# chellmuth/pathed

Measured on AMD Instinct MI355X. Metric: Msamples/s (pixels x spp / s), PathTracer radiance loop, higher is better.
Workload: dtype f32; 1 GPU; scenes/cornell.json 1024x1024, 1024 spp per step x 8 steps = 8192 spp, bounces 0..10, seed 1; total_samples=8589934592, parallelism=the samples of every step split over 1 GPU(s), no exchange

## Files before the change

pathed_amd/csrc/kernels.h:

```cpp
#pragma once

#ifndef PATHED_RESOLVE_SHARED
#define PATHED_RESOLVE_SHARED 2
#endif
#ifndef PATHED_EXPERIMENTS
#define PATHED_EXPERIMENTS 0
#endif
#include "mfma_candidates.h"
#include "small_items.h"
#include "camera_masks.h"
#include "shading.h"
#include "trace.h"
#include "volume.h"

namespace pathed {

static const int kBlock = 256;
static_assert(kBlock == kVolumeBlock, "volume.h indexes the LDS stack rows with the block size");
static const int kWavesPerBlock = kBlock / 64;
static const int kMaxLdsMaterials = 96;
#ifndef PATHED_UNIT_QUEUES
#define PATHED_UNIT_QUEUES 32
#endif
static const int kUnitQueues = PATHED_UNIT_QUEUES;
// ... 1115 lines not shown
                target = (unsigned int)floatAsInt(sd.w);
                valid = true;
            }
        }
        if (__ballot(valid) == 0ull) { continue; }

        unsigned int candidatesLow = 0, candidatesHigh = 0;
        if (valid) {
            smallCandidates<true>(smallTris.data, nTris, ray.o, ray.d, &candidatesLow, &candidatesHigh,
                                  candidateNear(ray.tnear), ray.anyHit ? candidateFar(ray.tfar) : 3e38f);
            if (COUNT) { trisTested += (unsigned int)nTris; }
        }

        smallResolve(geometry, ray, candidatesLow, candidatesHigh);

        if (valid) {
            finishRay(geometry, ray);
            if (ray.anyHit) {
                if (ray.occluded) { p.state.pend[target] = make_float4(0.f, 0.f, 0.f, 0.f); }
                if (COUNT) { shadowRays++; }
            } else {
                p.state.hit[target] = make_float4(ray.best, ray.bestU, ray.bestV, intAsFloat(ray.bestPrim));
                if (COUNT) { closestRays++; }
            }
        }
    }

    if (COUNT) {
        atomicAdd(&p.stats[kStatTris], (unsigned long long)trisTested);
        atomicAdd(&p.stats[kStatClosest], (unsigned long long)closestRays);
        atomicAdd(&p.stats[kStatShadow], (unsigned long long)shadowRays);
    }
}

template <int STACK, int FORMAT>
__global__ __launch_bounds__(kBlock) void k_trace_rays(
    DScene scene, const float4 *rays, int n, int anyHit, float4 *hitsOut, int *occludedOut,
    int *stackOverflow, int maxStack
) {
    extern __shared__ float4 ldsRaw[];
    LaneStack stack;
    stack.lds = reinterpret_cast<int *>(ldsRaw) + threadIdx.x;
    stack.overflowStride = (size_t)gridDim.x * kBlock;
    stack.overflow = stackOverflow + ((size_t)blockIdx.x * kBlock + threadIdx.x);

    TraceGeometry geometry;
    geometry.nodes = FORMAT != 0 ? scene.nodesQ : scene.nodes;
    geometry.tris = scene.leafTris;
    geometry.nNodes = scene.nNodes;
    geometry.nTris = scene.nTris;
    geometry.spheres = scene.spheres;
    geometry.nSpheres = scene.nLinearSpheres;

    const int i = blockIdx.x * kBlock + threadIdx.x;
    if (i >= n) { return; }
    const float4 ro = rays[2 * i + 0];
    const float4 rd = rays[2 * i + 1];
    RayHit hit;
    hit.t = 0.f; hit.u = 0.f; hit.v = 0.f; hit.prim = -1;
    TraceCounters counters;
    if (anyHit) {
        const bool occluded = traverse<false, STACK, kBlock, FORMAT>(
            geometry, stack, maxStack, v3(ro.x, ro.y, ro.z), v3(rd.x, rd.y, rd.z), ro.w, rd.w, true, &hit, &counters);
        occludedOut[i] = occluded ? 1 : 0;
    } else {
        const bool found = traverse<false, STACK, kBlock, FORMAT>(
            geometry, stack, maxStack, v3(ro.x, ro.y, ro.z), v3(rd.x, rd.y, rd.z), ro.w, rd.w, false, &hit, &counters);
        if (!found) { hit.t = 0.f; hit.u = 0.f; hit.v = 0.f; hit.prim = -1; }
        hitsOut[i] = make_float4(hit.t, hit.u, hit.v, intAsFloat(hit.prim));
    }
}

template <int STACK, bool COUNT>
__global__ __launch_bounds__(kBlock) void k_trace_instanced(RenderParams p, DInstanceSet instances)
{
    extern __shared__ float4 ldsRaw[];
    LaneStack stack;
    stack.lds = reinterpret_cast<int *>(ldsRaw) + threadIdx.x;
    stack.overflowStride = (size_t)gridDim.x * kBlock;
    stack.overflow = p.stackOverflow + ((size_t)blockIdx.x * kBlock + threadIdx.x);

    TraceGeometry geometry;
    geometry.nodes = p.scene.nodes;
    geometry.tris = p.scene.leafTris;
    geometry.nNodes = p.scene.nNodes;
    geometry.nTris = p.scene.nTris;
    geometry.spheres = nullptr;
    geometry.nSpheres = 0;

    const int lane = threadIdx.x & 63;
    const unsigned int waveId = blockIdx.x * kWavesPerBlock + (threadIdx.x >> 6);
    const unsigned int waveCount = gridDim.x * kWavesPerBlock;
    const unsigned int slotBatches = (unsigned int)p.nSlots / 64u;
    const unsigned int shadowCount = p.counters[kCtrShadowCount + (p.parity ^ 1) * kCursorStride];
    const unsigned int totalBatches = slotBatches + (shadowCount + 63u) / 64u;

    TraceCounters counters;
    counters.boxes = 0;
    counters.tris = 0;
    unsigned int closestRays = 0, shadowRays = 0;

    for (unsigned int batch = waveId; batch < totalBatches; batch += waveCount) {
        LaneRay ray;
        const float4 *worldO = nullptr, *worldD = nullptr;
        unsigned int target = 0;
        if (batch < slotBatches) {
            const unsigned int slot = batch * 64u + lane;
            const float4 rd = p.state.rayD[slot];
            if (!(floatAsInt(rd.w) & kStDone)) {
                const float4 ro = p.state.rayO[slot];
                laneRayInit(ray, v3(ro.x, ro.y, ro.z), v3(rd.x, rd.y, rd.z), PATHED_TNEAR, PATHED_TFAR, false);
                worldO = p.state.rayO + slot;
                worldD = p.state.rayD + slot;
                target = slot;
            }
        } else {
            const unsigned int entry = (batch - slotBatches) * 64u + lane;
            if (entry < shadowCount) {
                const float4 so = p.state.shO[entry];
                const float4 sd = p.state.shD[entry];
                laneRayInit(ray, v3(so.x, so.y, so.z), v3(sd.x, sd.y, sd.z), PATHED_TNEAR, so.w, true);
                worldO = p.state.shO + entry;
                worldD = p.state.shD + entry;
                target = (unsigned int)floatAsInt(sd.w);
            }
        }
        if (worldO == nullptr) { continue; }
        traverseInstanced<COUNT, STACK, kBlock>(geometry, instances, stack, p.maxStack, worldO, worldD, ray, &counters);
        if (ray.anyHit) {
            if (ray.occluded) { p.state.pend[target] = make_float4(0.f, 0.f, 0.f, 0.f); }
            if (COUNT) { shadowRays++; }
        } else {
            p.state.hit[target] = make_float4(ray.best, ray.bestU, ray.bestV, intAsFloat(ray.bestPrim));
            if (COUNT) { closestRays++; }
        }
    }

    if (COUNT) {
        atomicAdd(&p.stats[kStatBoxes], (unsigned long long)counters.boxes);
        atomicAdd(&p.stats[kStatTris], (unsigned long long)counters.tris);
        atomicAdd(&p.stats[kStatClosest], (unsigned long long)closestRays);
        atomicAdd(&p.stats[kStatShadow], (unsigned long long)shadowRays);
    }
}

template <int STACK>
__global__ __launch_bounds__(kBlock) void k_trace_rays_instanced(
    DScene scene, DInstanceSet instances, const float4 *rays, int n, int anyHit, float4 *hitsOut, int *occludedOut,
    int *stackOverflow, int maxStack
) {
    extern __shared__ float4 ldsRaw[];
    LaneStack stack;
    stack.lds = reinterpret_cast<int *>(ldsRaw) + threadIdx.x;
    stack.overflowStride = (size_t)gridDim.x * kBlock;
    stack.overflow = stackOverflow + ((size_t)blockIdx.x * kBlock + threadIdx.x);

    TraceGeometry geometry;
    geometry.nodes = scene.nodes;
    geometry.tris = scene.leafTris;
    geometry.nNodes = scene.nNodes;
    geometry.nTris = scene.nTris;
    geometry.spheres = nullptr;
    geometry.nSpheres = 0;

    const int i = blockIdx.x * kBlock + threadIdx.x;
    if (i >= n) { return; }
    const float4 ro = rays[2 * i + 0];
    const float4 rd = rays[2 * i + 1];
    TraceCounters counters;
    LaneRay ray;
    laneRayInit(ray, v3(ro.x, ro.y, ro.z), v3(rd.x, rd.y, rd.z), ro.w, rd.w, anyHit != 0);
    traverseInstanced<false, STACK, kBlock>(geometry, instances, stack, maxStack, rays + 2 * i, rays + 2 * i + 1, ray, &counters);
    if (anyHit) {
        occludedOut[i] = ray.occluded ? 1 : 0;
    } else if (ray.bestPrim >= 0) {
        hitsOut[i] = make_float4(ray.best, ray.bestU, ray.bestV, intAsFloat(ray.bestPrim));
    } else {
        hitsOut[i] = make_float4(0.f, 0.f, 0.f, intAsFloat(-1));
    }
}


__device__ inline V3 triangleNormal(V3 p0, V3 p1, V3 p2) { return normalized(xcross(p1 - p0, p2 - p0)); }

template <typename TRAITS = TraitsAll, bool INSTANCED = false>
__device__ inline Isect makeIsect(const DScene &scene, V3 o, V3 d, float4 h, const DInstanceSet *instances = nullptr)
{
    const float t = h.x, u = h.y, v = h.z;
#if defined(PATHED_ABLATE) && PATHED_ABLATE == 1
    const int prim = floatAsInt(h.w) & 1023;
#else
    const int prim = floatAsInt(h.w);
#endif

    V3 geometricNormal;
    V3 shadingNormal = v3(0.f, 0.f, 0.f);
    float uvU = 0.f, uvV = 0.f;
    int material;

    if (INSTANCED && prim >= instances->worldTris) {
        int low = 0, high = instances->nInstances - 1;
        while (low < high) {
            const int middle = (low + high + 1) >> 1;
            if (instances->bases[middle] <= prim) { low = middle; } else { high = middle - 1; }
        }
        const float4 *record = instances->records + (size_t)kInstanceQuads * low;
        const float4 m0 = record[0], m1 = record[1], m2 = record[2], i0 = record[3], i1 = record[4], i2 = record[5], ids = record[6];
        const float m[12] = { m0.x, m0.y, m0.z, m0.w, m1.x, m1.y, m1.z, m1.w, m2.x, m2.y, m2.z, m2.w };
        const float inverse[12] = { i0.x, i0.y, i0.z, i0.w, i1.x, i1.y, i1.z, i1.w, i2.x, i2.y, i2.z, i2.w };
        const float4 *q = scene.triShade + (size_t)kTriShadeQuads * (size_t)(floatAsInt(ids.w) + (prim - floatAsInt(ids.x)));
        const float4 q0 = q[0], q1 = q[1], q2 = q[2], q3 = q[3], q4 = q[4], q5 = q[5], q6 = q[6];
        const V3 p0 = flattenPoint(m, v3(q0.x, q0.y, q0.z)), p1 = flattenPoint(m, v3(q1.x, q1.y, q1.z)), p2 = flattenPoint(m, v3(q2.x, q2.y, q2.z));
        const V3 n0 = flattenNormal(inverse, v3(q3.x, q3.y, q3.z)), n1 = flattenNormal(inverse, v3(q4.x, q4.y, q4.z)), n2 = flattenNormal(inverse, v3(q5.x, q5.y, q5.z));
        const float w = 1.f - u - v;
        uvU = fmaf(w, q1.w, fmaf(u, q3.w, v * q5.w));
        uvV = fmaf(w, q2.w, fmaf(u, q4.w, v * q6.x));
        shadingNormal = v3(
            fmaf(w, n0.x, fmaf(u, n1.x, v * n2.x)),
            fmaf(w, n0.y, fmaf(u, n1.y, v * n2.y)),
            fmaf(w, n0.z, fmaf(u, n1.z, v * n2.z)));
        geometricNormal = triangleNormal(p0, p1, p2);
        material = floatAsInt(q0.w);
        if (length(shadingNormal) == 0.f) { shadingNormal = geometricNormal; }
        shadingNormal = normalized(shadingNormal);
    } else if (!TRAITS::spheres || prim < scene.nTris) {
        bool plain = false;
        for (int r = 0; r < scene.nPlainRanges; r++) { plain = plain || (prim >= scene.plainBegin[r] && prim < scene.plainEnd[r]); }
        if (plain) {
            const float4 *c = scene.triCompact + (size_t)kTriCompactQuads * prim;
            const float4 c0 = c[0], c1 = c[1];
            material = floatAsInt(c0.w);
            geometricNormal = v3(c0.x, c0.y, c0.z);
            shadingNormal = v3(c1.x, c1.y, c1.z);
        } else {
            const float4 *q = scene.triShade + (size_t)kTriShadeQuads * prim;
            const float4 q0 = q[0], q1 = q[1], q2 = q[2], q3 = q[3], q4 = q[4], q5 = q[5], q6 = q[6];
            const V3 p0 = v3(q0.x, q0.y, q0.z), p1 = v3(q1.x, q1.y, q1.z), p2 = v3(q2.x, q2.y, q2.z);
            const float w = 1.f - u - v;
            uvU = fmaf(w, q1.w, fmaf(u, q3.w, v * q5.w));
            uvV = fmaf(w, q2.w, fmaf(u, q4.w, v * q6.x));
            shadingNormal = v3(
                fmaf(w, q3.x, fmaf(u, q4.x, v * q5.x)),
                fmaf(w, q3.y, fmaf(u, q4.y, v * q5.y)),
                fmaf(w, q3.z, fmaf(u, q4.z, v * q5.z)));
            geometricNormal = triangleNormal(p0, p1, p2);
            material = floatAsInt(q0.w);
            if (length(shadingNormal) == 0.f) { shadingNormal = geometricNormal; }
            shadingNormal = normalized(shadingNormal);
        }
    } else {
        const DSphere sphere = scene.spheres[prim - scene.nTris];
        const V3 point = o + d * t;
        geometricNormal = normalized(point - v3(sphere.centerWorld[0], sphere.centerWorld[1], sphere.centerWorld[2]));
        material = sphere.material;
        shadingNormal = normalized(geometricNormal);
    }

    Isect isect;
    isect.point = o + d * t;
    isect.wo = -d;
    isect.normal = geometricNormal;
    isect.shadingNormal = shadingNormal;
    isect.u = uvU;
    isect.v = uvV;
    isect.material = material;
    isect.prim = prim;
    isect.frame = normalToWorldSpace(isect.shadingNormal, isect.wo);
    isect.woLocal = v3(__builtin_nanf(""), __builtin_nanf(""), __builtin_nanf(""));
    return isect;
}

template <typename TRAITS = TraitsAll>
__device__ inline float lightsPDF(const DScene &scene, V3 referencePoint, const Isect &lightIsect)
{
    float measurePDF;
    if (!TRAITS::spheres || lightIsect.prim < scene.nTris) {
        const float4 q7 = scene.triShade[(size_t)kTriShadeQuads * lightIsect.prim + 7];
        measurePDF = areaToSolidAngle(q7.w, referencePoint, lightIsect.point, v3(q7.x, q7.y, q7.z));
    } else {
        const DSphere sphere = scene.spheres[lightIsect.prim - scene.nTris];
        measurePDF = spherePdfSolidAngle(
            v3(sphere.centerSample[0], sphere.centerSample[1], sphere.centerSample[2]), sphere.radius, referencePoint);
    }
    return measurePDF / scene.nLights;
}

template <typename TRAITS = TraitsAll>
__device__ inline Rgb environmentL(const DScene &scene, V3 direction)
{
    if (!TRAITS::env) { return rgb(0.f); }
#if defined(PATHED_ABLATE) && PATHED_ABLATE == 3
    return rgb(0.f);
#endif
    if (scene.hasEnv) { return envEmit(scene.env, -direction); }
    return rgb(0.f);
}

struct ShadowRequest {
    bool push;
    V3 origin, direction;
    float tfar;
};

template <bool ENV_ONLY = false, typename TRAITS = TraitsAll, typename MaterialTable>
__device__ inline Rgb sampleLightsTerm(
    const DScene &scene, const MaterialTable &materials,
    const Isect &isect, const DMaterial &material, Rng &random, ShadowRequest *shadow
) {
    shadow->push = false;
#if defined(PATHED_ABLATE) && PATHED_ABLATE == 2
    return rgb(0.f);
#endif
    if (isDeltaT<TRAITS>(material)) { return rgb(0.f); }
    if (scene.nLights == 0) { return rgb(0.f); }

    const int lightCount = ENV_ONLY ? 1 : scene.nLights;
    DLight light;
    light.kind = 2;
    light.index = 0;
    int lightIndex = 0;
    if (ENV_ONLY) {
        random.dimension++;
    } else {
        lightIndex = (int)floorf(random.next() * lightCount);
        lightIndex = imin(lightIndex, lightCount - 1);
        light = scene.lights[lightIndex];
    }

    SurfaceSample surfaceSample;
    int lightMaterial = 0;
    constexpr bool kRecords = !ENV_ONLY && TRAITS::triangleLights && !TRAITS::spheres && !TRAITS::env;
    float pdfArea = 0.f;
    if (ENV_ONLY) {
        surfaceSample = envSample<TRAITS::pairedTrig>(scene.env, isect.point, random);
    } else if (!kRecords && TRAITS::triangleLights && light.kind == 0) {
        const float4 *q = scene.triShade + (size_t)kTriShadeQuads * light.index;
        const float4 q0 = q[0], q1 = q[1], q2 = q[2];
        surfaceSample = triangleSample(v3(q0.x, q0.y, q0.z), v3(q1.x, q1.y, q1.z), v3(q2.x, q2.y, q2.z), random);
        lightMaterial = floatAsInt(q0.w);
    } else if (kRecords) {
        const float4 *l = scene.lightRecords + (size_t)kLightRecordQuads * lightIndex;
        const float4 l0 = l[0], l1 = l[1], l2 = l[2];
        surfaceSample = triangleSamplePoint(v3(l0.x, l0.y, l0.z), v3(l1.x, l1.y, l1.z), v3(l2.x, l2.y, l2.z), v3(0.f, 0.f, 0.f), l1.w, random);
        __builtin_amdgcn_sched_barrier(0);
        const float4 l3 = l[3];
        surfaceSample.normal = v3(l3.x, l3.y, l3.z);
        lightMaterial = floatAsInt(l0.w);
        pdfArea = l3.w;
    } else if (TRAITS::spheres && (light.kind == 1 || !TRAITS::env)) {
        const DSphere sphere = scene.spheres[light.index];
        surfaceSample = sphereSample<TRAITS::pairedTrig>(
            v3(sphere.centerSample[0], sphere.centerSample[1], sphere.centerSample[2]), sphere.radius, isect.point, random);
        lightMaterial = sphere.material;
    } else if (TRAITS::env) {
        surfaceSample = envSample<TRAITS::pairedTrig>(scene.env, isect.point, random);
    } else {
        surfaceSample.point = isect.point;
        surfaceSample.normal = v3(0.f, 0.f, 0.f);
        surfaceSample.invPDF = 1.f;
        surfaceSample.solidAngle = 1;
    }
    const float lightChoicePDF = 1.f / lightCount;
    const float invPDF = surfaceSample.invPDF * (1.f / lightChoicePDF);
    if (!kRecords) { pdfArea = 1.f / invPDF; }

    const V3 lightDirection = surfaceSample.point - isect.point;
    const V3 wiWorld = normalized(lightDirection);

    if (dot(surfaceSample.normal, wiWorld) >= 0.f) { return rgb(0.f); }

    const float lightDistance = length(lightDirection);

    float pdf;
    if (surfaceSample.solidAngle) {
        pdf = pdfArea;
    } else {
        const V3 lightWoForPdf = -normalized(lightDirection);
        const float distance2 = lightDistance * lightDistance;
        const float projectedArea = smax(0.f, dot(surfaceSample.normal, lightWoForPdf));
        pdf = pdfArea * distance2 / projectedArea;
    }

    float brdfPDF;
    const Rgb f = materialF<TRAITS>(material, isect, wiWorld, &brdfPDF);
    const float lightWeight = (1 * pdf) / (1 * pdf + 1 * brdfPDF);

    if (isBlack(f) && pdf > 0.f && pdf < 3e38f && brdfPDF >= 0.f && brdfPDF < 3e38f) { return rgb(0.f); }

    const V3 lightWo = -normalized(lightDirection);
    Rgb emitted;
    if (ENV_ONLY || (TRAITS::env && light.kind == 2)) { emitted = envEmit(scene.env, lightWo); }
    else { emitted = matEmit(materials[lightMaterial]); }

    shadow->push = true;
    shadow->origin = isect.point;
    shadow->direction = wiWorld;
    shadow->tfar = lightDistance - 1e-3f;

    const Rgb contribution = emitted
        * lightWeight
        * f
        * fabsf(dot(isect.shadingNormal, wiWorld))
        / pdf;
    return contribution;
}

__device__ inline void startSample(const RenderParams &p, uint32_t pixel, uint32_t sample, int sampleInUnit, float4 *rayO, float4 *rayD)
{
    const int width = p.scene.camera.resX;
    const int row = (int)fastDivide((unsigned int)pixel, p.divWidth);
    const int col = (int)pixel - row * width;
    Rng random;
    makeKey(((uint64_t)p.seedHi << 32) | p.seedLo, pixel, sample, &random.k0, &random.k1);
    random.dimension = 0;
    const float jitterX = random.next() - 0.5f;
    const float jitterY = random.next() - 0.5f;
    V3 origin, direction;
    cameraRay(p.scene.camera, row + jitterY, col + jitterX, &origin, &direction);
    *rayO = make_float4(origin.x, origin.y, origin.z, intAsFloat(-1));
    *rayD = make_float4(direction.x, direction.y, direction.z, intAsFloat(sampleInUnit << kStSampleShift));
}

__device__ inline unsigned int grabUnits(const RenderParams &p, bool want, unsigned int *ldsScratch)
{
    const int lane = threadIdx.x & 63;
    const int wave = threadIdx.x >> 6;
    const unsigned int queues = (unsigned int)p.nQueues;
    const unsigned int home = blockIdx.x % queues;
    unsigned int mine = 0xFFFFFFFFu;
    for (unsigned int attempt = 0; attempt < queues; attempt++) {
        const unsigned long long mask = __ballot(want);
        const unsigned int before = (unsigned int)__popcll(mask & ((1ull << lane) - 1ull));
        if (lane == 0) { ldsScratch[wave] = (unsigned int)__popcll(mask); }
        __syncthreads();
        unsigned int offset = 0, total = 0;
        #pragma unroll
        for (int w = 0; w < kWavesPerBlock; w++) {
            const unsigned int count = ldsScratch[w];
            if (w < wave) { offset += count; }
            total += count;
        }
        if (total == 0u) { __syncthreads(); break; }
        const unsigned int queue = (unsigned int)__builtin_amdgcn_readfirstlane((int)(home + attempt < queues ? home + attempt : home + attempt - queues));
        const unsigned int limit = p.queueUnits[queue];
        if (threadIdx.x == 0) {
            unsigned int *cursor = &p.counters[kCtrUnitCursor + queue * kCursorStride];
            const unsigned int seen = __atomic_load_n(cursor, __ATOMIC_RELAXED);
            ldsScratch[kWavesPerBlock] = seen < limit ? atomicAdd(cursor, total) : 0xFFFFFFFFu;
        }
        __syncthreads();
        const unsigned int base = ldsScratch[kWavesPerBlock];
        __syncthreads();
        if (base >= limit) { continue; }
        if (want) {
            const unsigned int k = base + offset + before;
            if (k < limit) { mine = queue * p.unitsPerQueue + k; want = false; }
        }
        if (base + total <= limit) { break; }
    }
    return mine;
}

static const int kOrderStripes = 0, kOrderStripesTiled = 1, kOrderTiles = 2, kOrderList = 3;

__device__ inline unsigned int tileWalkPixel(const RenderParams &p, unsigned int index)
{
    const unsigned int width = (unsigned int)p.scene.camera.resX, height = (unsigned int)p.scene.camera.resY;
    const unsigned int band = fastDivide(index, p.divBand);
    const unsigned int inBand = index - band * 8u * width;
    const unsigned int rowsLeft = height - 8u * band;
    const unsigned int rows = rowsLeft < 8u ? rowsLeft : 8u;
    const unsigned int block = rows == 8u ? inBand >> 8 : inBand / (32u * rows);
    const unsigned int inBlock = inBand - block * 32u * rows;
    const unsigned int columnsLeft = width - 32u * block;
    const unsigned int columns = columnsLeft < 32u ? columnsLeft : 32u;
    const unsigned int y = columns == 32u ? inBlock >> 5 : inBlock / columns;
    const unsigned int x = inBlock - y * columns;
    return (8u * band + y) * width + 32u * block + x;
}

__device__ inline const uint32_t *pixelList(const RenderParams &p) { return reinterpret_cast<const uint32_t *>(p.cameraQueue); }

template <bool LIST = false>
__device__ inline void unitPlace(const RenderParams &p, unsigned int unit, uint32_t *pixel, uint32_t *chunkIndex)
{
    const unsigned int queue = fastDivide(unit, p.divStride);
    const unsigned int k = unit - queue * p.unitsPerQueue;
    const unsigned int j = fastDivide(k, p.divGroupUnits);
    const unsigned int w = k - j * p.groupUnits;
    const unsigned int owned = queue * p.pools + p.pool + j * (unsigned int)p.nQueues * p.pools;
    if (p.unitOrder != kOrderTiles) {
        *chunkIndex = owned;
        if constexpr (LIST) {
            if (p.unitOrder == kOrderStripes) { *pixel = w; }
            else if (p.unitOrder == kOrderList) { *pixel = pixelList(p)[w]; }
            else { *pixel = tileWalkPixel(p, w); }
        } else {
            *pixel = p.unitOrder == kOrderStripes ? w : tileWalkPixel(p, w);
        }
        return;
    }
    unsigned int chunk, within;
    if (owned + 1u < p.nGroups || p.lastGroupPixels == kUnitGroup) {
        chunk = w >> 8;
        within = w & (kUnitGroup - 1u);
    } else {
        chunk = w / p.lastGroupPixels;
        within = w - chunk * p.lastGroupPixels;
    }
    *pixel = tileWalkPixel(p, owned * kUnitGroup + within);
    *chunkIndex = chunk;
}

template <bool LIST = false>
__device__ inline void unitSamples(const RenderParams &p, unsigned int unit, uint32_t *pixel, uint32_t *first, uint32_t *end)
{
    uint32_t chunkIndex;
    unitPlace<LIST>(p, unit, pixel, &chunkIndex);
    *first = p.sppBegin + chunkIndex * (unsigned int)p.chunk;
    const uint32_t last = *first + (unsigned int)p.chunk;
    *end = last < p.sppEnd ? last : p.sppEnd;
}

template <bool LIST = false>
__device__ inline size_t partialIndex(const RenderParams &p, unsigned int unit)
{
    uint32_t pixel, chunkIndex;
    unitPlace<LIST>(p, unit, &pixel, &chunkIndex);
    return (size_t)chunkIndex * (size_t)p.nPixels + pixel;
}

__global__ __launch_bounds__(kBlock) void k_init(RenderParams p)
{
    __shared__ unsigned int scratch[kWavesPerBlock + 1];
    const int slot = blockIdx.x * kBlock + threadIdx.x;
    const unsigned int unit = grabUnits(p, true, scratch);

    float4 rayO = make_float4(0.f, 0.f, 0.f, intAsFloat(-1));
    float4 rayD = make_float4(0.f, 0.f, 0.f, intAsFloat(kStDone));
    const bool started = unit != 0xFFFFFFFFu;
    if (started) {
        uint32_t pixel, first, end;
        unitSamples<true>(p, unit, &pixel, &first, &end);
        startSample(p, pixel, first, 0, &rayO, &rayD);
    }
    p.state.rayO[slot] = rayO;
    p.state.rayD[slot] = rayD;
    p.state.res[slot] = make_float4(0.f, 0.f, 0.f, intAsFloat((int)unit));
    p.state.mod[slot] = make_float4(1.f, 1.f, 1.f, 1.f);
    p.state.thr[slot] = make_float4(0.f, 0.f, 0.f, 0.f);
    p.state.pend[slot] = make_float4(0.f, 0.f, 0.f, 0.f);
    p.state.acc[slot] = make_float4(0.f, 0.f, 0.f, 0.f);

    const unsigned long long mask = __ballot(started);
    if ((threadIdx.x & 63) == 0 && mask != 0ull) {
        atomicAdd(&p.counters[kCtrRemaining], (unsigned int)__popcll(mask));
    }
}

__global__ __launch_bounds__(kBlock) void k_resolve(RenderParams p)
{
    const int pixel = blockIdx.x * kBlock + threadIdx.x;
    if (pixel >= p.nPixels) { return; }
    float *out = p.accum + 3 * (size_t)pixel;
    float r = out[0], g = out[1], b = out[2];
    int chunk = 0;
    for (; chunk + 8 <= p.chunksPerPixel; chunk += 8) {
        float4 partial[8];
        #pragma unroll
        for (int k = 0; k < 8; k++) { partial[k] = p.state.chunkBuf[(size_t)(chunk + k) * p.nPixels + pixel]; }
        #pragma unroll
        for (int k = 0; k < 8; k++) {
            r += partial[k].x;
            g += partial[k].y;
            b += partial[k].z;
        }
    }
    for (; chunk < p.chunksPerPixel; chunk++) {
        const float4 partial = p.state.chunkBuf[(size_t)chunk * p.nPixels + pixel];
        r += partial.x;
        g += partial.y;
        b += partial.z;
    }
    out[0] = r;
    out[1] = g;
    out[2] = b;
}

struct MomentsParams {
    const float4 *chunkBuf;
    int nPixels;
    int chunksPerPixel;
    float *sum;
    float *squares;
};

__global__ __launch_bounds__(kBlock) void k_resolve_moments(MomentsParams p)
{
    const int pixel = blockIdx.x * kBlock + threadIdx.x;
    if (pixel >= p.nPixels) { return; }
    float *out = p.sum + 3 * (size_t)pixel;
    float *outSquares = p.squares + 3 * (size_t)pixel;
    float r = out[0], g = out[1], b = out[2];
    float rr = outSquares[0], gg = outSquares[1], bb = outSquares[2];
    int chunk = 0;
    for (; chunk + 8 <= p.chunksPerPixel; chunk += 8) {
        float4 partial[8];
        #pragma unroll
        for (int k = 0; k < 8; k++) { partial[k] = p.chunkBuf[(size_t)(chunk + k) * p.nPixels + pixel]; }
        #pragma unroll
// ... 725 lines not shown

    ShadowRequest shadow;
    shadow.push = false;
    shadow.origin = v3(0.f, 0.f, 0.f);
    shadow.direction = v3(0.f, 0.f, 0.f);
    shadow.tfar = 0.f;

    bool finished = false;
    Rgb color = rgb(0.f);
    unsigned int unit = 0xFFFFFFFFu;
    int sampleInUnit = 0;
    float4 outRayO = make_float4(0.f, 0.f, 0.f, 0.f), outRayD = rd;
    float4 outMod = make_float4(1.f, 1.f, 1.f, 1.f);
    float4 outThr = make_float4(0.f, 0.f, 0.f, 0.f);
    float4 outPend = make_float4(0.f, 0.f, 0.f, 0.f);
    Rgb result = rgb(0.f);
    V3 o = v3(0.f, 0.f, 0.f), d = v3(0.f, 0.f, 1.f);
    float4 hitNow = h;
    int rayBounce = 0, firstEmitMaterial = -1;
    uint32_t pixel = 0, sample = 0;
    bool haveVertex = false;
    bool hitWritten = false;
    float4 localHit = make_float4(PATHED_TFAR, 0.f, 0.f, intAsFloat(-1));

    unsigned int countedClosest = 0u, countedShadow = 0u;

    SHADE_REGION(0, true);
    SHADE_REGION(1, active);
    if (active) {
        const float4 ro = roIn;
        const float4 resIn = resIn0;
        outRayO = ro;
        o = v3(ro.x, ro.y, ro.z);
        d = v3(rd.x, rd.y, rd.z);
        rayBounce = st & kStBounceMask;
        sampleInUnit = (st >> kStSampleShift) & kStSampleMask;
        const bool miss = floatAsInt(h.w) < 0;
        unit = (unsigned int)floatAsInt(resIn.w);
        firstEmitMaterial = floatAsInt(ro.w);
        uint32_t firstSample, endSample;
        unitSamples<true>(p, unit, &pixel, &firstSample, &endSample);
        sample = firstSample + (uint32_t)sampleInUnit;
        result = rgb(resIn.x, resIn.y, resIn.z);
        Rgb modulation = rgb(1.f);
        Rgb missLight = rgb(0.f);
        if (miss && (rayBounce == 0 || (st & kStEligible))) { missLight = environmentL<TRAITS>(scene, d); }

        if (rayBounce == 0) {
            if (miss) {
                color = rgb(0.f) + missLight;
                finished = true;
            } else {
                firstEmitMaterial = -1;
                result = rgb(0.f);
                haveVertex = true;
            }
        } else {
            const float4 modIn = p.state.mod[slot];
            const float4 thrIn = p.state.thr[slot];
            modulation = rgb(modIn.x, modIn.y, modIn.z);
            const float bsdfPdf = modIn.w;
            const Rgb throughput = rgb(thrIn.x, thrIn.y, thrIn.z);
            const float cosTheta = thrIn.w;
            if (st & kStEligible) {
                Rgb bsdfTerm = rgb(0.f);
                if (miss) {
                    const Rgb environmentLight = missLight;
                    if (!isBlack(environmentLight)) {
                        const float lightPDF = envEmitPDF(scene.env, d) / 1;
                        const float brdfWeight = (st & kStDelta)
                            ? 1.f
                            : (1 * bsdfPdf) / (1 * bsdfPdf + 1 * lightPDF);
                        bsdfTerm = environmentLight * brdfWeight * throughput * cosTheta / bsdfPdf;
                    }
                }
                const Rgb Ld = rgb(pendIn.x, pendIn.y, pendIn.z) + bsdfTerm;
                if (rayBounce == 1) { result = Ld; }
                else { result = result + Ld * modulation; }
            }
            if (!(st & kStContinue) || miss) {
                finished = true;
            } else {
                const float invPDF = 1.f / bsdfPdf;
                modulation = modulation * (throughput * cosTheta * invPDF);
                if (isBlack(modulation)) { finished = true; }
                else { haveVertex = true; }
            }
            if (finished) {
                const Rgb first = rgb(0.f);
                color = first + result;
            }
        }
        outMod = make_float4(modulation.r, modulation.g, modulation.b, 1.f);
    }

    bool retiredAny = false;
#define PATHED_END_OF_SAMPLE(ended, value, startedNext, nextPixel, nextSample)                                                 \
    {                                                                                                                        \
        bool needUnit_ = false;                                                                                              \
        startedNext = false;                                                                                                 \
        SHADE_REGION(7, ended);                                                                                              \
        if (ended) {                                                                                                         \
            const bool singleSample_ = PATHED_SHADE_TRIM && p.chunk == 1;                                                    \
            float4 partial_ = make_float4(0.f, 0.f, 0.f, 0.f);                                                               \
            if (!singleSample_) { partial_ = p.state.acc[slot]; }                                                            \
            const bool finite_ = isfinite((value).r) && isfinite((value).g) && isfinite((value).b);                          \
            if (finite_) {                                                                                                   \
                partial_.x += (value).r;                                                                                     \
                partial_.y += (value).g;                                                                                     \
                partial_.z += (value).b;                                                                                     \
            } else {                                                                                                         \
                atomicAdd(&p.stats[kStatDropped], 1ull);                                                                     \
            }                                                                                                                \
            uint32_t unitPixel_, firstSample_, endSample_;                                                                   \
            unitSamples<true>(p, unit, &unitPixel_, &firstSample_, &endSample_);                                             \
            sampleInUnit++;                                                                                                  \
            result = rgb(0.f);                                                                                               \
            outMod = make_float4(1.f, 1.f, 1.f, 1.f);                                                                        \
            outThr = make_float4(0.f, 0.f, 0.f, 0.f);                                                                        \
            outPend = make_float4(0.f, 0.f, 0.f, 0.f);                                                                       \
            if (firstSample_ + (uint32_t)sampleInUnit < endSample_) {                                                        \
                startedNext = true;                                                                                          \
                nextPixel = unitPixel_;                                                                                      \
                nextSample = firstSample_ + (uint32_t)sampleInUnit;                                                          \
                p.state.acc[slot] = partial_;                                                                                \
            } else {                                                                                                         \
                p.state.chunkBuf[partialIndex<true>(p, unit)] = partial_;                                                    \
                if (!singleSample_) { p.state.acc[slot] = make_float4(0.f, 0.f, 0.f, 0.f); }                                 \
                needUnit_ = true;                                                                                            \
            }                                                                                                                \
        }                                                                                                                    \
        const unsigned int newUnit_ = grabUnits(p, needUnit_, scratch);                                                      \
        if (needUnit_) {                                                                                                     \
            unit = newUnit_;                                                                                                 \
            if (newUnit_ != 0xFFFFFFFFu) {                                                                                   \
                uint32_t endSample_;                                                                                         \
                unitSamples<true>(p, newUnit_, &nextPixel, &nextSample, &endSample_);                                        \
                sampleInUnit = 0;                                                                                            \
                startedNext = true;                                                                                          \
            } else {                                                                                                         \
                outRayD.w = intAsFloat(kStDone);                                                                             \
                retiredAny = true;                                                                                           \
            }                                                                                                                \
        }                                                                                                                    \
        SHADE_REGION(8, startedNext);                                                                                        \
        if (startedNext) { startSample(p, nextPixel, nextSample, sampleInUnit, &outRayO, &outRayD); }                        \
    }

    {
        bool startedNext;
        uint32_t nextPixel = 0, nextSample = 0;
        PATHED_END_OF_SAMPLE(active && finished, color, startedNext, nextPixel, nextSample)
        if (p.localCount > 0) {
            const V3 cameraO = v3(outRayO.x, outRayO.y, outRayO.z), cameraD = v3(outRayD.x, outRayD.y, outRayD.z);
            const bool localCamera = startedNext && !localMeetsRest(p, cameraO, cameraD, PATHED_TFAR);
            const float4 found = localClosestHit(p, localCamera, cameraO, cameraD);
            if (localCamera) {
                countedClosest++;
                if (floatAsInt(found.w) >= 0) {
                    o = cameraO; d = cameraD; hitNow = found;
                    rayBounce = 0; firstEmitMaterial = -1;
                    pixel = nextPixel; sample = nextSample;
                    result = rgb(0.f);
                    haveVertex = true;
                } else {
                    localHit = found;
                    hitWritten = true;
                    outRayD.w = intAsFloat(floatAsInt(outRayD.w) | kStLocal);
                }
            }
        }
    }

    SHADE_REGION(5, haveVertex);
    if (haveVertex) {
        Isect isect = makeIsect<TRAITS>(scene, o, d, hitNow);
        const int vertex = rayBounce + 1;
        const DMaterial &material = materials[isect.material];
        prepareLobes<TRAITS>(material, isect);
        Rng random;
        makeKey(((uint64_t)p.seedHi << 32) | p.seedLo, pixel, sample, &random.k0, &random.k1);
        random.dimension = vertexBase(vertex);
        const BSDFSample bsdfSample = materialSample<TRAITS>(material, isect, random);

        const bool counts = checkCounts(p.startBounce, p.lastBounce, vertex);
        const bool wantDirect = counts;
        const bool wantContinue = !checkDone(p.lastBounce, vertex + 1);

        Rgb lightTerm = rgb(0.f);
        SHADE_REGION(6, wantDirect);
        if (wantDirect) {
            random.dimension = vertexBase(vertex) + 3;
            lightTerm = sampleLightsTerm<true, TRAITS>(scene, materials, isect, material, random, &shadow);
        }
        const bool deadEnd = isBlack(bsdfSample.throughput) && bsdfSample.pdf > 0.f && bsdfSample.pdf < 3e38f
            && !shadow.push && isBlack(lightTerm);
        if ((!wantDirect && !wantContinue) || deadEnd) {
            outRayO = make_float4(isect.point.x, isect.point.y, isect.point.z, intAsFloat(firstEmitMaterial));
            outRayD = make_float4(d.x, d.y, d.z, intAsFloat((vertex | (sampleInUnit << kStSampleShift)) | kStLocal));
            outMod.w = 1.f;
            outThr = make_float4(0.f, 0.f, 0.f, 0.f);
            outPend = make_float4(0.f, 0.f, 0.f, 0.f);
            localHit = make_float4(PATHED_TFAR, 0.f, 0.f, intAsFloat(-1));
            hitWritten = true;
            shadow.push = false;
        } else {
            int nextState = vertex | (sampleInUnit << kStSampleShift);
            if (wantDirect) { nextState |= kStEligible; }
            if (isDeltaT<TRAITS>(material)) { nextState |= kStDelta; }
            if (wantContinue) { nextState |= kStContinue; }
            outRayO = make_float4(isect.point.x, isect.point.y, isect.point.z, intAsFloat(firstEmitMaterial));
            outRayD = make_float4(bsdfSample.wiWorld.x, bsdfSample.wiWorld.y, bsdfSample.wiWorld.z, intAsFloat(nextState));
            if (rayBounce == 0) { outMod = make_float4(1.f, 1.f, 1.f, 1.f); }
            outMod.w = bsdfSample.pdf;
            outThr = make_float4(
                bsdfSample.throughput.r, bsdfSample.throughput.g, bsdfSample.throughput.b,
                fabsf(dot(isect.shadingNormal, bsdfSample.wiWorld)));
            outPend = make_float4(lightTerm.r, lightTerm.g, lightTerm.b, 0.f);
            hitWritten = false;
        }
    }
#undef PATHED_END_OF_SAMPLE

    if (p.localCount > 0) {
        const bool retiredNow = (floatAsInt(outRayD.w) & kStDone) != 0;
        const bool hasRay = active && !retiredNow;
        const V3 nextO = v3(outRayO.x, outRayO.y, outRayO.z), nextD = v3(outRayD.x, outRayD.y, outRayD.z);
        const bool localClosest = hasRay && !hitWritten && !localMeetsRest(p, nextO, nextD, PATHED_TFAR);
        const bool localShadow = shadow.push && !localMeetsRest(p, shadow.origin, shadow.direction, shadow.tfar);
        {
            const float4 found = localClosestHit(p, localClosest, nextO, nextD);
            if (localClosest) {
                localHit = found;
                hitWritten = true;
                outRayD.w = intAsFloat(floatAsInt(outRayD.w) | kStLocal);
                countedClosest++;
            }
            const bool occluded = localOccluded(p, localShadow, shadow.origin, shadow.direction, shadow.tfar);
            if (localShadow) {
                if (occluded) { outPend = make_float4(0.f, 0.f, 0.f, 0.f); }
                shadow.push = false;
                countedShadow++;
            }
        }
        if (hasRay && (!(floatAsInt(outRayD.w) & kStLocal) || shadow.push)) { outRayD.w = intAsFloat(floatAsInt(outRayD.w) | kStAwait); }
        if (p.localCounting) {
            for (int offset = 32; offset >= 1; offset >>= 1) {
                countedClosest += (unsigned int)__shfl_xor((int)countedClosest, offset, 64);
                countedShadow += (unsigned int)__shfl_xor((int)countedShadow, offset, 64);
            }
            if (lane == 0 && (countedClosest | countedShadow) != 0u) {
                atomicAdd(&p.stats[kStatLocalClosest], (unsigned long long)countedClosest);
                atomicAdd(&p.stats[kStatLocalShadow], (unsigned long long)countedShadow);
            }
        }
    }

    if (active) {
        p.state.rayO[slot] = outRayO;
        p.state.rayD[slot] = outRayD;
        p.state.res[slot] = make_float4(result.r, result.g, result.b, intAsFloat((int)unit));
        if (hitWritten) { p.state.hit[slot] = localHit; }
        p.state.mod[slot] = outMod;
        p.state.thr[slot] = outThr;
        p.state.pend[slot] = outPend;
    }

    {
        const unsigned long long mask = __ballot(shadow.push);
        const unsigned int before = (unsigned int)__popcll(mask & ((1ull << lane) - 1ull));
        if (lane == 0) { scratch[wave] = (unsigned int)__popcll(mask); }
        __syncthreads();
        unsigned int offset = 0, total = 0;
        #pragma unroll
        for (int w = 0; w < kWavesPerBlock; w++) {
            const unsigned int count = scratch[w];
            if (w < wave) { offset += count; }
            total += count;
        }
        __syncthreads();
        if (threadIdx.x == 0) {
            scratch[kWavesPerBlock] = total ? atomicAdd(&p.counters[kCtrShadowCount + p.parity * kCursorStride], total) : 0u;
        }
        __syncthreads();
        if (shadow.push) {
            const unsigned int index = scratch[kWavesPerBlock] + offset + before;
            p.state.shO[index] = make_float4(shadow.origin.x, shadow.origin.y, shadow.origin.z, shadow.tfar);
            p.state.shD[index] = make_float4(shadow.direction.x, shadow.direction.y, shadow.direction.z, intAsFloat(slot));
        }
    }

    const unsigned long long retiredMask = __ballot(retiredAny);
    if (lane == 0 && retiredMask != 0ull) {
        atomicSub(&p.counters[kCtrRemaining], (unsigned int)__popcll(retiredMask));
    }
}

#ifndef PATHED_FUSED_WAVES
#define PATHED_FUSED_WAVES 4
#endif
template <bool LDS_MATERIALS, bool COUNT, typename TRAITS, bool MFMA = false, bool QUADS = false>
__global__ __launch_bounds__(kBlock) __attribute__((amdgpu_waves_per_eu(PATHED_FUSED_WAVES, PATHED_FUSED_WAVES))) void k_path_small(RenderParams p, SmallTris smallTris)
{
    extern __shared__ float4 ldsDynamic[];
    __shared__ float mfmaRows[MFMA ? kMfmaTableFloats : 1];
    __shared__ float4 stashRows[QUADS ? 6 * kBlock : 1];
    constexpr int kResolveCapacity = PATHED_RESOLVE_SHARED == 2 ? 128 : 64;
    __shared__ unsigned long long resolveBest[QUADS ? kBlock : 1];
    __shared__ float2 resolveUv[QUADS ? kWavesPerBlock * kResolveCapacity : 1];
    __shared__ unsigned short resolveItems[QUADS ? kWavesPerBlock * kResolveCapacity : 1];
    __shared__ unsigned int resolveOccluded[QUADS ? kBlock : 1], resolveCount[QUADS ? kWavesPerBlock : 1];
    if (MFMA) {
        for (int i = threadIdx.x; i < kMfmaTableFloats; i += kBlock) { mfmaRows[i] = p.mfmaTable[i]; }
        if (!LDS_MATERIALS) { __syncthreads(); }
    }
    const MaterialAccess<LDS_MATERIALS> materials = stageMaterials<LDS_MATERIALS>(p, ldsDynamic);
    const TraceGeometry geometry = sceneGeometry(p.scene, false);

    const DScene &scene = p.scene;
    const int lane = threadIdx.x & 63;
    const unsigned int waveId = blockIdx.x * kWavesPerBlock + (unsigned int)__builtin_amdgcn_readfirstlane((int)(threadIdx.x >> 6));
    const int nTris = p.scene.nTris;
    constexpr bool kPassList = QUADS && kSmallPassList<COUNT, MFMA, TRAITS>;
    TraceGeometry passGeometry = geometry;
    if (kPassList) { passGeometry.tris = geometry.tris + 3 * nTris; }
    const uint64_t seed = ((uint64_t)p.seedHi << 32) | p.seedLo;
    UnitTaker units(p, waveId);

    bool alive = true;
    bool needEntry = true;
    unsigned int unit = 0xFFFFFFFFu;
    uint32_t pixel = 0, sample = 0, endSample = 0;
    PathRegisters path = idlePath();
    float4 partial = make_float4(0.f, 0.f, 0.f, 0.f);
    bool pendingShadow = false;
    V3 shadowDirection = v3(0.f, 0.f, 1.f);
    float shadowTfar = 0.f;

    unsigned int closestRays = 0, shadowRays = 0, trisTested = 0;

    float4 *const cameraQueue = p.cameraQueue + (size_t)waveId * kCameraQueueWords;
    unsigned int queueHead = 0u, queueCount = 0u;
    bool unitsLeft = true;
    const bool singleSample = p.chunk == 1;

    bool startNext = false;

    while (true) {
        SHADE_REGION(0, alive && !needEntry);
        SHADE_REGION(1, startNext);
        if (startNext) {
            startCameraSample(p, seed, pixel, sample, path);
            startNext = false;
        }

        if (QUADS) {
            float4 *stash = stashRows + threadIdx.x;
            stash[0 * kBlock] = make_float4(path.result.r, path.result.g, path.result.b, path.bsdfPdf);
            stash[1 * kBlock] = make_float4(path.modulation.r, path.modulation.g, path.modulation.b, path.cosTheta);
            stash[2 * kBlock] = make_float4(path.throughput.r, path.throughput.g, path.throughput.b, intAsFloat(path.st));
            stash[3 * kBlock] = partial;
            stash[4 * kBlock] = make_float4(intAsFloat((int)pixel), intAsFloat((int)sample), intAsFloat((int)endSample), intAsFloat((int)unit));
            stash[5 * kBlock] = make_float4(intAsFloat((int)path.random.k0), intAsFloat((int)path.random.k1), intAsFloat(path.firstEmitMaterial), intAsFloat((int)path.random.dimension));
            asm volatile("" ::: "memory");
        }

        if (queueCount < 64u && unitsLeft) {
            const unsigned int newUnit = units.take(p, lane, true);
            const bool got = newUnit != 0xFFFFFFFFu;
            const unsigned long long gotMask = __ballot(got);
            SHADE_REGION(11, got);
            if (gotMask != ~0ull) { unitsLeft = false; }
            Rng cameraRandom;
            cameraRandom.k0 = 0u; cameraRandom.k1 = 0u; cameraRandom.dimension = 0u;
            V3 cameraO = v3(0.f, 0.f, 0.f), cameraD = v3(0.f, 0.f, 1.f);
            constexpr bool kMasks = !COUNT && !MFMA;
            uint32_t unitPixel = 0u;
            if (got) {
                uint32_t unitFirst, unitEnd;
                unitSamples(p, newUnit, &unitPixel, &unitFirst, &unitEnd);
                cameraSampleRay(p, seed, unitPixel, unitFirst, cameraRandom, &cameraO, &cameraD);
            }
            LaneRay cameraHit;
            laneRayInit(cameraHit, cameraO, cameraD, PATHED_TNEAR, PATHED_TFAR, false);
            unsigned int candidatesLow = 0, candidatesHigh = 0;
            if (kMasks) {
                if (got) {
                    const unsigned long long pixelCandidates = cameraMasks(p)[unitPixel];
                    candidatesLow = (unsigned int)(pixelCandidates >> 32);
                    candidatesHigh = (unsigned int)pixelCandidates;
                }
            } else if (got) {
                if (QUADS || MFMA) {
                    unsigned int unusedLow = 0, unusedHigh = 0;
                    smallCandidatesItems<false, true, true>(smallTris.data, p.smallQuads, nTris, p.smallKappaT, cameraO, cameraD, cameraD,
                                                             &candidatesLow, &candidatesHigh, &unusedLow, &unusedHigh, candidateNear(PATHED_TNEAR), 0.f);
                } else {
                    smallCandidates(smallTris.data, nTris, cameraO, cameraD, &candidatesLow, &candidatesHigh, candidateNear(PATHED_TNEAR));
                }
            }
            if (COUNT && got) {
                trisTested += (unsigned int)nTris;
                closestRays++;
            }
            smallResolve(geometry, cameraHit, candidatesLow, candidatesHigh);
            if (got) {
                finishRay(geometry, cameraHit);
                const unsigned int slot = (queueHead + queueCount + laneRank(gotMask)) & (kCameraQueueEntries - 1u);
                const unsigned int target = singleSample ? (unsigned int)partialIndex(p, newUnit) : newUnit;
                cameraQueue[0 * kCameraQueueEntries + slot] = make_float4(cameraD.x, cameraD.y, cameraD.z, cameraHit.best);
                cameraQueue[1 * kCameraQueueEntries + slot] = make_float4(cameraHit.bestU, cameraHit.bestV, intAsFloat(cameraHit.bestPrim), intAsFloat((int)target));
                cameraQueue[2 * kCameraQueueEntries + slot] = make_float4(intAsFloat((int)cameraRandom.k0), intAsFloat((int)cameraRandom.k1), 0.f, 0.f);
            }
            queueCount += (unsigned int)__popcll(gotMask);
            __threadfence_block();
        }

        const bool tracing = alive && !needEntry;
        LaneRay ray;
        laneRayInit(ray, path.o, path.d, PATHED_TNEAR, PATHED_TFAR, false);
        {
            const bool traceShadow = tracing && pendingShadow;
            LaneRay shadowRay;
            laneRayInit(shadowRay, path.o, shadowDirection, PATHED_TNEAR, shadowTfar, true);
            unsigned int candidatesLow = 0, candidatesHigh = 0, shadowLow = 0, shadowHigh = 0;
            SHADE_REGION(2, traceShadow);
            if (MFMA) {
                mfmaCandidatesPair(mfmaRows, nTris, p.mfmaFrame, __ballot(traceShadow) != 0ull, path.o, path.d, shadowDirection,
                                   candidateNear(PATHED_TNEAR), candidateFar(shadowTfar), &candidatesLow, &candidatesHigh, &shadowLow, &shadowHigh);
                if (!tracing) { candidatesLow = 0u; candidatesHigh = 0u; }
                if (!traceShadow) { shadowLow = 0u; shadowHigh = 0u; }
            } else if (QUADS) {
                if (tracing) {
                    constexpr bool kPrune = kSmallPrunes<COUNT, TRAITS>;
                    const int smallQuads = kPassList ? (p.smallQuads & 0xFF) : kPrune ? (p.smallQuads & 0xFFFF) : p.smallQuads;
                    const int passTris = kPassList ? ((p.smallQuads >> 8) & 0xFF) : nTris;
                    smallCandidatesItems<true, true, true, kPrune>(smallTris.data, smallQuads, passTris, p.smallKappaT, path.o, path.d, shadowDirection,
                                                                   &candidatesLow, &candidatesHigh, &shadowLow, &shadowHigh,
                                                                   candidateNear(PATHED_TNEAR), candidateFar(shadowTfar),
                                                                   (p.smallQuads >> 16) & 0xFF, (p.smallQuads >> 24) & 0xFF);
                    if (!traceShadow) { shadowLow = 0u; shadowHigh = 0u; }
                }
            } else if (__ballot(traceShadow) != 0ull) {
                if (tracing) {
                    smallCandidatesPair(smallTris.data, nTris, path.o, path.d, shadowDirection, &candidatesLow, &candidatesHigh, &shadowLow, &shadowHigh,
                                        candidateNear(PATHED_TNEAR), candidateFar(shadowTfar));
                    if (!traceShadow) { shadowLow = 0u; shadowHigh = 0u; }
                }
            } else if (tracing) {
                smallCandidates(smallTris.data, nTris, path.o, path.d, &candidatesLow, &candidatesHigh, candidateNear(PATHED_TNEAR));
            }
            if (COUNT && tracing) {
                trisTested += (unsigned int)nTris * (traceShadow ? 2u : 1u);
                closestRays++;
                if (traceShadow) { shadowRays++; }
            }
            bool spheresDone = false;
            RESOLVE_PROBE(9, candidatesLow, candidatesHigh);
            RESOLVE_PROBE(10, shadowLow, shadowHigh);
            if (MFMA) {
                mfmaResolve(geometry, ray, candidatesLow, candidatesHigh);
                mfmaResolve(geometry, shadowRay, shadowLow, shadowHigh);
            } else if (QUADS && PATHED_RESOLVE_SHARED) {
                ResolveScratch scratch;
                const int waveBase = (int)(threadIdx.x & ~63u), wave = (int)(threadIdx.x >> 6);
                scratch.best = resolveBest + waveBase; scratch.uv = resolveUv + wave * kResolveCapacity; scratch.items = resolveItems + wave * kResolveCapacity;
                scratch.occluded = resolveOccluded + waveBase; scratch.count = resolveCount + wave;
                unsigned int sphereCandidates = 0u, shadowSphereCandidates = 0u;
                if (TRAITS::spheres && geometry.nSpheres > 0 && tracing) {
                    smallSphereCandidates(p, geometry.nSpheres, path.o, path.d, shadowDirection, &sphereCandidates, &shadowSphereCandidates);
                    if (!traceShadow) { shadowSphereCandidates = 0u; }
                }
                spheresDone = smallResolveShared<kResolveCapacity, PATHED_RESOLVE_SHARED != 2, TRAITS::spheres>(
                    passGeometry, ray, shadowRay, candidatesLow, candidatesHigh, shadowLow, shadowHigh, sphereCandidates, shadowSphereCandidates, scratch);
            } else {
                smallResolve(passGeometry, ray, candidatesLow, candidatesHigh);
                smallResolve(passGeometry, shadowRay, shadowLow, shadowHigh);
            }
            if (tracing && !spheresDone) { finishRay(geometry, ray); }
            if (traceShadow) {
                if (!spheresDone) { finishRay(geometry, shadowRay); }
                if (shadowRay.occluded) { path.pend = rgb(0.f); }
            }
            pendingShadow = false;
        }
        if (QUADS) {
            asm volatile("" ::: "memory");
            const float4 *stash = stashRows + threadIdx.x;
            const float4 s0 = stash[0 * kBlock], s1 = stash[1 * kBlock], s2 = stash[2 * kBlock], s4 = stash[4 * kBlock], s5 = stash[5 * kBlock];
            path.result = rgb(0.f); path.result.r = s0.x; path.result.g = s0.y; path.result.b = s0.z; path.bsdfPdf = s0.w;
            path.modulation.r = s1.x; path.modulation.g = s1.y; path.modulation.b = s1.z; path.cosTheta = s1.w;
            path.throughput.r = s2.x; path.throughput.g = s2.y; path.throughput.b = s2.z; path.st = floatAsInt(s2.w);
            partial = stash[3 * kBlock];
            pixel = (uint32_t)floatAsInt(s4.x); sample = (uint32_t)floatAsInt(s4.y); endSample = (uint32_t)floatAsInt(s4.z); unit = (unsigned int)floatAsInt(s4.w);
            path.random.k0 = (uint32_t)floatAsInt(s5.x); path.random.k1 = (uint32_t)floatAsInt(s5.y); path.firstEmitMaterial = floatAsInt(s5.z); path.random.dimension = (uint32_t)floatAsInt(s5.w);
        }
        float4 h = make_float4(ray.best, ray.bestU, ray.bestV, intAsFloat(ray.bestPrim));

        bool done = false;
        bool departs = false;
        Rgb color = rgb(0.f);
        if (tracing) {
            const bool miss = floatAsInt(h.w) < 0;
            Isect arrived;
            SHADE_REGION(3, !miss);
            if (!miss) { arrived = makeIsect<TRAITS>(scene, path.o, path.d, h); }
            done = pathArrive<TRAITS, true>(p, scene, materials, path, arrived, miss, &color);
            departs = !done;
        }

        while (true) {
            SHADE_REGION(8, done);
            {
                const bool unitDone = putSampleAway(p, singleSample, done, color, partial, unit, sample, endSample);
                needEntry = needEntry || unitDone;
                startNext = startNext || (done && !unitDone);
            }
            done = false;
            const unsigned long long wanting = __ballot(needEntry);
            if (wanting == 0ull) { break; }
            if (queueCount == 0u) {
                if (!unitsLeft && needEntry) { alive = false; needEntry = false; }
                break;
            }
            __threadfence_block();
            const unsigned int rank = laneRank(wanting);
            if (needEntry && rank < queueCount) {
                const unsigned int slot = (queueHead + rank) & (kCameraQueueEntries - 1u);
                const float4 e0 = cameraQueue[0 * kCameraQueueEntries + slot];
                const float4 e1 = cameraQueue[1 * kCameraQueueEntries + slot];
                const float4 e2 = cameraQueue[2 * kCameraQueueEntries + slot];
                resetPath(path);
                path.o = cameraOrigin(scene.camera);
                path.d = v3(e0.x, e0.y, e0.z);
                path.random.k0 = (uint32_t)floatAsInt(e2.x); path.random.k1 = (uint32_t)floatAsInt(e2.y); path.random.dimension = 2u;
                h = make_float4(e0.w, e1.x, e1.y, e1.z);
                unit = (unsigned int)floatAsInt(e1.w);
                if (singleSample) { sample = 0u; endSample = 1u; }
                else { unitSamples(p, unit, &pixel, &sample, &endSample); }
                needEntry = false;
                if (floatAsInt(h.w) < 0) {
                    color = cameraMissColor<TRAITS>(scene, path.d);
                    done = true;
                } else {
                    departs = true;
                }
            }
            const unsigned int wanted = (unsigned int)__popcll(wanting);
            const unsigned int taken = wanted < queueCount ? wanted : queueCount;
            queueHead = (queueHead + taken) & (kCameraQueueEntries - 1u);
            queueCount -= taken;
        }
        if (__ballot(alive) == 0ull) { break; }

        SHADE_REGION(6, departs);
        bool ended = false;
        if (departs) {
            Isect isect = makeIsect<TRAITS>(scene, path.o, path.d, h);
            ShadowRequest shadow;
            ended = pathDepart<TRAITS, true>(p, scene, materials, path, isect, &shadow, &color);
            if (shadow.push) {
                pendingShadow = true;
                shadowDirection = shadow.direction;
                shadowTfar = shadow.tfar;
            }
        }
        if (__ballot(ended) != 0ull) {
            SHADE_REGION(8, ended);
            const bool unitDone = putSampleAway(p, singleSample, ended, color, partial, unit, sample, endSample);
            needEntry = needEntry || unitDone;
            startNext = startNext || (ended && !unitDone);
        }
    }

    if (COUNT) {
        atomicAdd(&p.stats[kStatTris], (unsigned long long)trisTested);
        atomicAdd(&p.stats[kStatClosest], (unsigned long long)closestRays);
        atomicAdd(&p.stats[kStatShadow], (unsigned long long)shadowRays);
    }
}

#include "path_wave.h"
#include "path_hybrid.h"
static_assert(sizeof(RenderParams) + sizeof(SmallTris) <= 4096, "the fused kernels' arguments must fit the 4 KB kernarg segment");

__global__ __launch_bounds__(kBlock) void k_debug_small_candidates(DScene scene, SmallTris smallTris, SmallTris smallItems, int nQuads, float kappaT,
                                                                   const float4 *itemTris, const float *mfmaTable, MfmaFrame frame,
                                                                   const float *rays, int n, unsigned long long *out)
{
#if PATHED_EXPERIMENTS
    __shared__ float mfmaRows[kMfmaTableFloats];
    for (int i = threadIdx.x; i < kMfmaTableFloats; i += kBlock) { mfmaRows[i] = mfmaTable[i]; }
    __syncthreads();
#endif
    const int index = blockIdx.x * kBlock + threadIdx.x;
    const float *r = rays + (size_t)10 * index;
    const V3 o = v3(r[0], r[1], r[2]), dA = v3(r[3], r[4], r[5]), dB = v3(r[6], r[7], r[8]);
    const float tfarB = r[9];
    const int nTris = scene.nTris;

    unsigned int aLow, aHigh, bLow, bHigh;
    smallCandidatesPair(smallTris.data, nTris, o, dA, dB, &aLow, &aHigh, &bLow, &bHigh, candidateNear(PATHED_TNEAR), candidateFar(tfarB));
    unsigned int iaLow, iaHigh, ibLow, ibHigh;
    smallCandidatesItems<true>(smallItems.data, nQuads, nTris, kappaT, o, dA, dB, &iaLow, &iaHigh, &ibLow, &ibHigh, candidateNear(PATHED_TNEAR), candidateFar(tfarB));
    unsigned int evenA = 0u, oddA = 0u, evenB = 0u, oddB = 0u;
#if PATHED_EXPERIMENTS
    mfmaCandidatesPair(mfmaRows, nTris, frame, true, o, dA, dB, candidateNear(PATHED_TNEAR), candidateFar(tfarB), &evenA, &oddA, &evenB, &oddB);
#endif

    unsigned long long valuA = 0, valuB = 0, mfmaA = 0, mfmaB = 0, acceptA = 0, acceptB = 0, itemsA = 0, itemsB = 0;
    for (int k = 0; k < nTris; k++) {
        const float4 t0 = scene.leafTris[3 * k + 0], t1 = scene.leafTris[3 * k + 1], t2 = scene.leafTris[3 * k + 2];
        const unsigned long long bit = 1ull << (floatAsInt(t0.w) & 63);
        if (((k < 32 ? aLow : aHigh) >> (31 - (k & 31))) & 1u) { valuA |= bit; }
        if (((k < 32 ? bLow : bHigh) >> (31 - (k & 31))) & 1u) { valuB |= bit; }
        if ((((k & 1) ? oddA : evenA) >> (k >> 1)) & 1u) { mfmaA |= bit; }
        if ((((k & 1) ? oddB : evenB) >> (k >> 1)) & 1u) { mfmaB |= bit; }
        float t, u, v;
        if (intersectTriangle(o, dA, v3(t0.x, t0.y, t0.z), v3(t1.x, t1.y, t1.z), v3(t2.x, t2.y, t2.z), &t, &u, &v) && t > PATHED_TNEAR && t <= PATHED_TFAR) { acceptA |= bit; }
        if (intersectTriangle(o, dB, v3(t0.x, t0.y, t0.z), v3(t1.x, t1.y, t1.z), v3(t2.x, t2.y, t2.z), &t, &u, &v) && t > PATHED_TNEAR && t <= tfarB) { acceptB |= bit; }
        const unsigned long long itemBit = 1ull << (floatAsInt(itemTris[3 * k].w) & 63);
        if (((k < 32 ? iaLow : iaHigh) >> (31 - (k & 31))) & 1u) { itemsA |= itemBit; }
        if (((k < 32 ? ibLow : ibHigh) >> (31 - (k & 31))) & 1u) { itemsB |= itemBit; }
    }
    if (index < n) {
        unsigned long long *row = out + (size_t)8 * index;
        row[0] = valuA; row[1] = valuB; row[2] = mfmaA; row[3] = mfmaB; row[4] = acceptA; row[5] = acceptB; row[6] = itemsA; row[7] = itemsB;
    }
}

__global__ __launch_bounds__(kBlock) void k_debug_shadow_candidates(DScene scene, SmallTris smallItems, int nQuads, float kappaT, int shadowQuadPairs, int shadowLonePairs,
                                                                    const float4 *itemTris, const float *rays, int n, unsigned long long *out)
{
    const int index = blockIdx.x * kBlock + threadIdx.x;
    const float *r = rays + (size_t)10 * index;
    const V3 o = v3(r[0], r[1], r[2]), dA = v3(r[3], r[4], r[5]), dB = v3(r[6], r[7], r[8]);
    const float tfarB = r[9];
    const int nTris = scene.nTris;
    unsigned int aLow, aHigh, bLow, bHigh;
    smallCandidatesItems<true, true, true, true>(smallItems.data, nQuads, nTris, kappaT, o, dA, dB, &aLow, &aHigh, &bLow, &bHigh,
                                                 candidateNear(PATHED_TNEAR), candidateFar(tfarB), shadowQuadPairs, shadowLonePairs);
    unsigned long long candidates = 0, accepted = 0;
    for (int k = 0; k < nTris; k++) {
        const float4 t0 = itemTris[3 * k + 0], t1 = itemTris[3 * k + 1], t2 = itemTris[3 * k + 2];
        const unsigned long long bit = 1ull << (floatAsInt(t0.w) & 63);
        if (((k < 32 ? bLow : bHigh) >> (31 - (k & 31))) & 1u) { candidates |= bit; }
        float t, u, v;
        if (intersectTriangle(o, dB, v3(t0.x, t0.y, t0.z), v3(t1.x, t1.y, t1.z), v3(t2.x, t2.y, t2.z), &t, &u, &v) && t > PATHED_TNEAR && t <= tfarB) { accepted |= bit; }
    }
    if (index < n) { out[(size_t)2 * index] = candidates; out[(size_t)2 * index + 1] = accepted; }
}

__global__ __launch_bounds__(kBlock) void k_debug_pass_candidates(SmallTris passItems, int nQuads, int nPass, float kappaT, int shadowQuadPairs, int shadowLonePairs,
                                                                  const float4 *passTris, const float *rays, int n, unsigned long long *out)
{
    const int index = blockIdx.x * kBlock + threadIdx.x;
    const float *r = rays + (size_t)10 * index;
    const V3 o = v3(r[0], r[1], r[2]), dA = v3(r[3], r[4], r[5]), dB = v3(r[6], r[7], r[8]);
    const float tfarB = r[9];
    unsigned int aLow, aHigh, bLow, bHigh;
    smallCandidatesItems<true, true, true, true>(passItems.data, nQuads, nPass, kappaT, o, dA, dB, &aLow, &aHigh, &bLow, &bHigh,
                                                 candidateNear(PATHED_TNEAR), candidateFar(tfarB), shadowQuadPairs, shadowLonePairs);
    unsigned long long candidatesA = 0, candidatesB = 0;
    for (int k = 0; k < nPass; k++) {
        const unsigned long long bit = 1ull << (floatAsInt(passTris[3 * k].w) & 63);
        if (((k < 32 ? aLow : aHigh) >> (31 - (k & 31))) & 1u) { candidatesA |= bit; }
        if (((k < 32 ? bLow : bHigh) >> (31 - (k & 31))) & 1u) { candidatesB |= bit; }
    }
    if (index < n) { out[(size_t)2 * index] = candidatesA; out[(size_t)2 * index + 1] = candidatesB; }
}

template <bool QUADS = false, typename MaterialTable>
__device__ __forceinline__ bool volumeQuerySmall(const VolumeContext<MaterialTable> &c, const f2 *pairRecords, int smallQuads, float smallKappaT,
                                                 int mode, V3 o, V3 d, float tfar, RayHit *hit, VolumeEvents *eventsOut)
{
    LaneRay ray;
    const bool anyHit = mode == kQueryVolumeOccluded;
    laneRayInit(ray, o, d, PATHED_TNEAR, tfar, anyHit);
    VolumeEvents events;
    eventsClear(events);
    unsigned int low = 0u, high = 0u;
    if (QUADS) {
        unsigned int unusedLow = 0u, unusedHigh = 0u;
        smallCandidatesItems<true>(pairRecords, smallQuads, c.geometry.nTris, smallKappaT, o, d, d, &unusedLow, &unusedHigh, &low, &high,
                                   candidateNear(PATHED_TNEAR), anyHit ? candidateFar(tfar) : 3e38f);
    } else {
        smallCandidates<true>(pairRecords, c.geometry.nTris, o, d, &low, &high, candidateNear(PATHED_TNEAR), anyHit ? candidateFar(tfar) : 3e38f);
    }
    bool decided = false;
    while (__ballot((low | high) != 0u) != 0ull) {
        if ((low | high) != 0u) {
            int k;
            if (low != 0u) { k = __clz((int)low); low &= ~(0x80000000u >> k); }
            else { k = __clz((int)high); high &= ~(0x80000000u >> k); k += 32; }
            const float4 t0 = c.geometry.tris[3 * k + 0];
            const float4 t1 = c.geometry.tris[3 * k + 1];
            const float4 t2 = c.geometry.tris[3 * k + 2];
            float t, u, v;
            if (intersectTriangle(ray.o, ray.d, v3(t0.x, t0.y, t0.z), v3(t1.x, t1.y, t1.z), v3(t2.x, t2.y, t2.z), &t, &u, &v)) {
                if (volumeAccept(c, mode, ray, events, t, u, v, floatAsInt(t0.w))) { decided = true; low = 0u; high = 0u; }
            }
        }
    }
    if (!decided) {
        for (int i = 0; i < c.geometry.nSpheres; i++) {
            if (volumeSphere(c, mode, ray, events, i)) { break; }
        }
    }
    if (mode == kQueryVolumeClosest) { eventsClip(events, ray.best); }
    if (eventsOut) { *eventsOut = events; }
    if (anyHit) { return ray.occluded; }
    hit->t = ray.best;
    hit->u = ray.bestU;
    hit->v = ray.bestV;
    hit->prim = ray.bestPrim;
    return ray.bestPrim >= 0;
}


template <bool QUADS = false, typename MaterialTable>
__device__ __forceinline__ void volumeQueryPairSmall(const VolumeContext<MaterialTable> &c, const f2 *pairRecords, int smallQuads, float smallKappaT, V3 o,
                                                     bool wantA, int modeA, V3 dA, RayHit *hitA, bool *foundA, VolumeEvents *eventsA,
                                                     bool wantB, V3 dB, float tfarB, bool *occludedB, VolumeEvents *eventsB)
{
    unsigned int lowA = 0u, highA = 0u, lowB = 0u, highB = 0u;
    if (QUADS) {
        smallCandidatesItems<true>(pairRecords, smallQuads, c.geometry.nTris, smallKappaT, o, dA, dB, &lowA, &highA, &lowB, &highB,
                                   candidateNear(PATHED_TNEAR), candidateFar(tfarB));
    } else {
        smallCandidatesPair(pairRecords, c.geometry.nTris, o, dA, dB, &lowA, &highA, &lowB, &highB, candidateNear(PATHED_TNEAR), candidateFar(tfarB));
    }
    if (!wantA) { lowA = 0u; highA = 0u; }
    if (!wantB) { lowB = 0u; highB = 0u; }
    auto resolve = [&](int mode, LaneRay &ray, VolumeEvents &events, unsigned int low, unsigned int high, bool want) {
        bool decided = false;
        while (__ballot((low | high) != 0u) != 0ull) {
            if ((low | high) != 0u) {
                int k;
                if (low != 0u) { k = __clz((int)low); low &= ~(0x80000000u >> k); }
                else { k = __clz((int)high); high &= ~(0x80000000u >> k); k += 32; }
                const float4 t0 = c.geometry.tris[3 * k + 0];
                const float4 t1 = c.geometry.tris[3 * k + 1];
                const float4 t2 = c.geometry.tris[3 * k + 2];
                float t, u, v;
                if (intersectTriangle(ray.o, ray.d, v3(t0.x, t0.y, t0.z), v3(t1.x, t1.y, t1.z), v3(t2.x, t2.y, t2.z), &t, &u, &v)) {
                    if (volumeAccept(c, mode, ray, events, t, u, v, floatAsInt(t0.w))) { decided = true; low = 0u; high = 0u; }
                }
            }
        }
        if (want && !decided) {
            for (int i = 0; i < c.geometry.nSpheres; i++) {
                if (volumeSphere(c, mode, ray, events, i)) { break; }
            }
        }
    };
    {
        LaneRay ray;
        laneRayInit(ray, o, dA, PATHED_TNEAR, PATHED_TFAR, false);
        VolumeEvents events;
        eventsClear(events);
        resolve(modeA, ray, events, lowA, highA, wantA);
        if (modeA == kQueryVolumeClosest) { eventsClip(events, ray.best); }
        *eventsA = events;
        hitA->t = ray.best; hitA->u = ray.bestU; hitA->v = ray.bestV; hitA->prim = ray.bestPrim;
        *foundA = ray.bestPrim >= 0;
    }
    {
        LaneRay ray;
        laneRayInit(ray, o, dB, PATHED_TNEAR, tfarB, true);
        VolumeEvents events;
        eventsClear(events);
        resolve(kQueryVolumeOccluded, ray, events, lowB, highB, wantB);
        *eventsB = events;
        *occludedB = ray.occluded;
    }
}

#ifndef PATHED_VOLUME_WAVES
#define PATHED_VOLUME_WAVES 4
#endif
template <bool LDS_MATERIALS, int STACK, bool SMALL, typename TRAITS, bool QUADS, bool GRID, bool MULTI = false, bool LIST = false>
__device__ __forceinline__ void pathVolume(const RenderParams &p, const SmallTris &smallTris)
{
    extern __shared__ float4 ldsRaw[];
    const MaterialAccess<LDS_MATERIALS> materials = stageMaterials<LDS_MATERIALS>(p, ldsRaw + ((STACK + 1) * kBlock) / 4);

    const DScene &scene = p.scene;
    VolumeContext<MaterialAccess<LDS_MATERIALS>> context;
    context.geometry = sceneGeometry(scene, true);
    context.stack.lds = reinterpret_cast<int *>(ldsRaw) + threadIdx.x;
    context.stack.overflowStride = (size_t)gridDim.x * kBlock;
    context.stack.overflow = p.stackOverflow + ((size_t)blockIdx.x * kBlock + threadIdx.x);
    context.maxStack = p.maxStack;
    context.scene = &scene;
    context.materials = materials;
    context.primMedium = scene.primMedium;
    context.media = scene.media;

    const int lane = threadIdx.x & 63;
    const unsigned int waveId = blockIdx.x * kWavesPerBlock + (threadIdx.x >> 6);
    const uint64_t seed = ((uint64_t)p.seedHi << 32) | p.seedLo;

    UnitTaker units(p, waveId);

    auto query = [&](int mode, V3 origin, V3 direction, float tfar, RayHit *hit, VolumeEvents *events) -> bool {
        if constexpr (SMALL) { return volumeQuerySmall<QUADS>(context, (const f2 *)smallTris.data, p.smallQuads, p.smallKappaT, mode, origin, direction, tfar, hit, events); }
        else { return volumeQuery<STACK>(context, mode, origin, direction, tfar, hit, events); }
    };

    auto transmit = [&](int index, V3 pointA, V3 pointB) -> Rgb {
        if constexpr (GRID) {
            const DMedium &record = context.media[index];
            if (record.kind == kMediumGrid) {
                const float channel = gridTransmittance(scene.grids[record.grid], scene.gridData, pointA, pointB);
                return rgb(channel, channel, channel);
            }
        }
        return mediumTransmittance(context.media[index], pointA, pointB);
    };
    auto transmission = [&](V3 origin, V3 direction, const VolumeEvents &events, int medium) -> Rgb {
        if constexpr (GRID) { return rayTransmissionOver(transmit, origin, direction, events, medium); }
        else { return rayTransmission(context.media, origin, direction, events, medium); }
    };

    RayHit segmentHit;
    segmentHit.t = 0.f; segmentHit.u = 0.f; segmentHit.v = 0.f; segmentHit.prim = -1;
    bool segmentFound = false, segmentKnown = false;

    auto vertexLighting = [&](const Isect &isect, int medium, const DMaterial &material, const BSDFSample &bsdfSample, Rng &random,
                              bool direct, bool needSegment) -> Rgb {
        SHADE_REGION(5, direct);
        const bool lit = direct && material.type != PATHED_MAT_PASSTHROUGH && isBlack(matEmit(material));
        bool wantShadow = false;
        DLight light;
        light.kind = 0; light.index = 0;
        SurfaceSample surfaceSample;
        surfaceSample.point = isect.point; surfaceSample.normal = v3(0.f, 0.f, 0.f); surfaceSample.invPDF = 1.f; surfaceSample.solidAngle = 1;
        int lightMaterial = 0;
        float invPDF = 1.f, lightDistance = 0.f;
        V3 lightDirection = v3(0.f, 0.f, 0.f), wiWorld = bsdfSample.wiWorld;
        if (lit && !volumeIsDelta(material) && scene.nLights != 0) {
            const int lightCount = scene.nLights;
            int lightIndex = (int)floorf(random.next() * lightCount);
            lightIndex = imin(lightIndex, lightCount - 1);
            light = scene.lights[lightIndex];
            if (TRAITS::triangleLights && light.kind == 0) {
                const LightRecord record = loadLightRecord(scene.lightRecords, lightIndex);
                surfaceSample = triangleSamplePoint(record.p0, record.p1, record.p2, record.normal, record.area, random);
                lightMaterial = record.material;
            } else if (TRAITS::spheres && light.kind == 1) {
                const DSphere sphere = scene.spheres[light.index];
                surfaceSample = sphereSample<TRAITS::pairedTrig>(v3(sphere.centerSample[0], sphere.centerSample[1], sphere.centerSample[2]), sphere.radius, isect.point, random);
                lightMaterial = sphere.material;
            } else if (TRAITS::env) {
                surfaceSample = envSample<TRAITS::pairedTrig>(scene.env, isect.point, random);
            } else {
                surfaceSample.point = isect.point; surfaceSample.normal = v3(0.f, 0.f, 0.f); surfaceSample.invPDF = 1.f; surfaceSample.solidAngle = 1;
            }
            const float lightChoicePDF = 1.f / lightCount;
            invPDF = surfaceSample.invPDF * (1.f / lightChoicePDF);
            lightDirection = surfaceSample.point - isect.point;
            wiWorld = normalized(lightDirection);
            if (!(dot(surfaceSample.normal, wiWorld) >= 0.f)) {
                lightDistance = length(lightDirection);
                wantShadow = true;
            }
        }

        const bool wantClosest = lit || needSegment;
        const int closestMode = lit ? kQueryVolumeClosest : kQueryRegular;
        RayHit bounceHit;
        bounceHit.t = 0.f; bounceHit.u = 0.f; bounceHit.v = 0.f; bounceHit.prim = -1;
        bool found = false, occluded = false;
        VolumeEvents skipped, events;
        eventsClear(skipped);
        eventsClear(events);
        auto finishLight = [&]() -> Rgb {
            if (!wantShadow || occluded) { return rgb(0.f); }
            const Rgb transmittance = transmission(isect.point, wiWorld, events, medium);
            float pdf;
            if (surfaceSample.solidAngle) {
                pdf = 1.f / invPDF;
// ... 603 lines not shown
```

pathed_amd/csrc/path_common.h:

```cpp

template <bool LDS_MATERIALS>
__device__ __forceinline__ MaterialAccess<LDS_MATERIALS> stageMaterials(const RenderParams &p, void *lds)
{
    MaterialAccess<LDS_MATERIALS> materials;
    if (LDS_MATERIALS) {
        const int words = p.scene.nMaterials * (int)(sizeof(DMaterial) / 4);
        const int *source = reinterpret_cast<const int *>(p.scene.materials);
        int *target = reinterpret_cast<int *>(lds);
        for (int i = threadIdx.x; i < words; i += kBlock) { target[i] = source[i]; }
        __syncthreads();
        materials.table = reinterpret_cast<const DMaterial *>(lds);
    } else {
        materials.table = p.scene.materials;
    }
    return materials;
}

__device__ __forceinline__ TraceGeometry sceneGeometry(const DScene &scene, bool tree)
{
    TraceGeometry geometry;
    geometry.nodes = tree ? scene.nodes : nullptr;
    geometry.tris = scene.leafTris;
    geometry.nNodes = tree ? scene.nNodes : 0;
    geometry.nTris = scene.nTris;
    geometry.spheres = scene.spheres;
    geometry.nSpheres = scene.nLinearSpheres;
    return geometry;
}

struct UnitTaker {
    unsigned int queue, queuesTried;
    unsigned int reservedNext, reservedEnd;

    __device__ __forceinline__ UnitTaker(const RenderParams &p, unsigned int waveId)
        : queue(waveId % (unsigned int)p.nQueues), queuesTried(0), reservedNext(0), reservedEnd(0) {}

    __device__ __forceinline__ unsigned int take(const RenderParams &p, int lane, bool want)
    {
        unsigned int mine = 0xFFFFFFFFu;
        unsigned long long wanting = __ballot(want);
        while (wanting != 0ull) {
            if (reservedNext == reservedEnd) {
                if (queuesTried >= (unsigned int)p.nQueues) { break; }
                unsigned int ticket = 0;
                if (lane == 0) { ticket = atomicAdd(&p.counters[kCtrUnitCursor + queue * kCursorStride], (unsigned int)p.unitGrab); }
                ticket = (unsigned int)__builtin_amdgcn_readfirstlane((int)ticket);
                const unsigned int limit = p.queueUnits[queue];
                if (ticket >= limit) {
                    queue = (queue + 1u) % (unsigned int)p.nQueues;
                    queuesTried++;
                    continue;
                }
                reservedNext = ticket;
                reservedEnd = ticket + (unsigned int)p.unitGrab < limit ? ticket + (unsigned int)p.unitGrab : limit;
            }
            const unsigned int available = reservedEnd - reservedNext;
            const unsigned int rank = laneRank(wanting);
            const bool served = ((wanting >> lane) & 1ull) != 0ull && rank < available;
            if (served) { mine = queue * p.unitsPerQueue + reservedNext + rank; }
            const unsigned int count = (unsigned int)__popcll(wanting);
            reservedNext += count < available ? count : available;
            wanting &= ~__ballot(served);
        }
        return mine;
    }
};

struct PathRegisters {
    V3 o, d;
    int st;
    int firstEmitMaterial;
    Rgb result, modulation, throughput, pend;
    float bsdfPdf, cosTheta;
    Rng random;
};

__device__ __forceinline__ void resetPath(PathRegisters &path)
{
    path.st = 0;
    path.firstEmitMaterial = -1;
    path.result = rgb(0.f);
    path.modulation = rgb(1.f);
    path.throughput = rgb(0.f);
    path.pend = rgb(0.f);
    path.bsdfPdf = 1.f;
    path.cosTheta = 0.f;
}

__device__ __forceinline__ PathRegisters idlePath()
{
    PathRegisters path;
    path.random.k0 = 0u; path.random.k1 = 0u; path.random.dimension = 0u;
    path.o = v3(0.f, 0.f, 0.f); path.d = v3(0.f, 0.f, 1.f);
    resetPath(path);
    return path;
}

__device__ __forceinline__ void cameraSampleRay(const RenderParams &p, uint64_t seed, uint32_t pixel, uint32_t sample, Rng &random, V3 *origin, V3 *direction)
{
    makeKey(seed, pixel, sample, &random.k0, &random.k1);
    random.dimension = 0;
    const int width = p.scene.camera.resX;
    const int row = (int)fastDivide((unsigned int)pixel, p.divWidth);
    const int col = (int)pixel - row * width;
    const float jitterX = random.next() - 0.5f;
    const float jitterY = random.next() - 0.5f;
    cameraRay(p.scene.camera, row + jitterY, col + jitterX, origin, direction);
}

__device__ __forceinline__ void startCameraSample(const RenderParams &p, uint64_t seed, uint32_t pixel, uint32_t sample, PathRegisters &path)
{
    cameraSampleRay(p, seed, pixel, sample, path.random, &path.o, &path.d);
    resetPath(path);
}


template <typename TRAITS>
__device__ __forceinline__ Rgb cameraMissColor(const DScene &scene, V3 direction)
{
    return rgb(0.f) + environmentL<TRAITS>(scene, direction);
}

template <typename TRAITS, bool PROBES = false, typename MATERIALS>
__device__ __forceinline__ bool pathArrive(const RenderParams &p, const DScene &scene, const MATERIALS &materials, PathRegisters &path, const Isect &isect,
                                           bool miss, Rgb *color)
{
    bool finished = false;
    *color = rgb(0.f);
    const int st = path.st;
    const int rayBounce = st & kStBounceMask;
    if (rayBounce == 0) {
        if (miss) {
            *color = cameraMissColor<TRAITS>(scene, path.d);
            finished = true;
        }
    } else {
        if (st & kStEligible) {
            Rgb bsdfTerm = rgb(0.f);
            if (!miss) {
                const Rgb emit = matEmit(materials[isect.material]);
                if (PROBES) { SHADE_REGION(5, !isBlack(emit) && dot(isect.wo, isect.shadingNormal) >= 0.f); }
                if (!isBlack(emit) && dot(isect.wo, isect.shadingNormal) >= 0.f) {
                    const float lightPDF = lightsPDF<TRAITS>(scene, path.o, isect);
                    const float brdfWeight = (st & kStDelta)
                        ? 1.f
                        : (1 * path.bsdfPdf) / (1 * path.bsdfPdf + 1 * lightPDF);
                    bsdfTerm = emit * brdfWeight * path.throughput * path.cosTheta / path.bsdfPdf;
                }
            } else {
                const Rgb environmentLight = environmentL<TRAITS>(scene, path.d);
                if (TRAITS::env && !isBlack(environmentLight)) {
                    const float lightPDF = envEmitPDF(scene.env, path.d) / scene.nLights;
                    const float brdfWeight = (st & kStDelta)
                        ? 1.f
                        : (1 * path.bsdfPdf) / (1 * path.bsdfPdf + 1 * lightPDF);
                    bsdfTerm = environmentLight * brdfWeight * path.throughput * path.cosTheta / path.bsdfPdf;
                }
            }
            const Rgb Ld = path.pend + bsdfTerm;
            if (rayBounce == 1) { path.result = Ld; }
            else { path.result = path.result + Ld * path.modulation; }
        }

        if (!(st & kStContinue) || miss) {
            finished = true;
        } else {
            const float invPDF = 1.f / path.bsdfPdf;
            path.modulation = path.modulation * (path.throughput * path.cosTheta * invPDF);
            if (isBlack(path.modulation)) { finished = true; }
        }
        if (finished) {
            Rgb first = rgb(0.f);
            if (path.firstEmitMaterial >= 0) { first = first + matEmit(materials[path.firstEmitMaterial]); }
            *color = first + path.result;
        }
    }
    return finished;
}

template <typename TRAITS, bool PROBES = false, typename MATERIALS>
__device__ __forceinline__ bool pathDepart(const RenderParams &p, const DScene &scene, const MATERIALS &materials, PathRegisters &path,
                                           Isect &isect, ShadowRequest *shadowOut, Rgb *color)
{
    ShadowRequest shadow;
    shadow.push = false;
    shadow.origin = v3(0.f, 0.f, 0.f);
    shadow.direction = v3(0.f, 0.f, 1.f);
    shadow.tfar = 0.f;
    bool finished = false;
    *color = rgb(0.f);
    const int rayBounce = path.st & kStBounceMask;
    const int vertex = rayBounce + 1;

    if (PROBES) { SHADE_REGION(4, rayBounce == 0); }
    if (rayBounce == 0) {
        path.firstEmitMaterial = -1;
        if (checkCounts(p.startBounce, p.lastBounce, 0)) {
            const Rgb emit = matEmit(materials[isect.material]);
            const bool backside = dot(isect.normal, isect.wo) < 0.f;
            if (!isBlack(emit) && !backside) { path.firstEmitMaterial = isect.material; }
        }
        path.result = rgb(0.f);
    }

    {
        const DMaterial &material = materials[isect.material];
        prepareLobes<TRAITS>(material, isect);

        path.random.dimension = vertexBase(vertex);
        const BSDFSample bsdfSample = materialSample<TRAITS>(material, isect, path.random);

        const bool counts = checkCounts(p.startBounce, p.lastBounce, vertex);
        const bool emissive = !isBlack(matEmit(material));
        const bool wantDirect = counts && !emissive;
        const bool wantContinue = !checkDone(p.lastBounce, vertex + 1);

        Rgb lightTerm = rgb(0.f);
        if (PROBES) { SHADE_REGION(7, wantDirect); }
        if (wantDirect) {
            path.random.dimension = vertexBase(vertex) + 3;
            lightTerm = sampleLightsTerm<false, TRAITS>(scene, materials, isect, material, path.random, &shadow);
        }

        const bool deadEnd = isBlack(bsdfSample.throughput) && bsdfSample.pdf > 0.f && bsdfSample.pdf < 3e38f
            && !shadow.push && isBlack(lightTerm);
        if ((!wantDirect && !wantContinue) || deadEnd) {
            finished = true;
            Rgb first = rgb(0.f);
            if (path.firstEmitMaterial >= 0) { first = first + matEmit(materials[path.firstEmitMaterial]); }
            *color = first + path.result;
            shadow.push = false;
        } else {
            int nextState = vertex;
            if (wantDirect) { nextState |= kStEligible; }
            if (isDeltaT<TRAITS>(material)) { nextState |= kStDelta; }
            if (wantContinue) { nextState |= kStContinue; }
            path.st = nextState;
            path.o = isect.point;
            path.d = bsdfSample.wiWorld;
            path.bsdfPdf = bsdfSample.pdf;
            path.throughput = bsdfSample.throughput;
            path.cosTheta = fabsf(dot(isect.shadingNormal, bsdfSample.wiWorld));
            path.pend = lightTerm;
        }
    }
    *shadowOut = shadow;
    return finished;
}

template <typename TRAITS, typename MATERIALS>
__device__ __forceinline__ bool pathVertex(const RenderParams &p, const DScene &scene, const MATERIALS &materials, PathRegisters &path,
                                           float4 h, ShadowRequest *shadowOut, Rgb *color)
{
    const bool miss = floatAsInt(h.w) < 0;
    Isect isect;
    if (!miss) { isect = makeIsect<TRAITS>(scene, path.o, path.d, h); }
    shadowOut->push = false;
    shadowOut->origin = v3(0.f, 0.f, 0.f);
    shadowOut->direction = v3(0.f, 0.f, 1.f);
    shadowOut->tfar = 0.f;
    if (pathArrive<TRAITS>(p, scene, materials, path, isect, miss, color)) { return true; }
    return pathDepart<TRAITS>(p, scene, materials, path, isect, shadowOut, color);
}

__device__ __forceinline__ void firstUnits(const RenderParams &p, UnitTaker &units, int lane, unsigned int &unit,
                                           uint32_t &pixel, uint32_t &sample, uint32_t &endSample, bool &alive, bool &startNext)
{
    unit = units.take(p, lane, true);
    if (unit != 0xFFFFFFFFu) {
        unitSamples(p, unit, &pixel, &sample, &endSample);
        alive = true;
        startNext = true;
    }
}

__device__ __forceinline__ bool putSampleAway(const RenderParams &p, bool unitIsIndex, bool done, Rgb color, float4 &partial, unsigned int unit,
                                              uint32_t &sample, uint32_t endSample)
{
    bool unitDone = false;
    if (done) {
        const bool finite = isfinite(color.r) && isfinite(color.g) && isfinite(color.b);
        if (finite) {
            partial.x += color.r;
            partial.y += color.g;
            partial.z += color.b;
        } else {
            atomicAdd(&p.stats[kStatDropped], 1ull);
        }
        sample++;
        if (sample >= endSample) {
            p.state.chunkBuf[unitIsIndex ? (size_t)unit : partialIndex(p, unit)] = partial;
            partial = make_float4(0.f, 0.f, 0.f, 0.f);
            unitDone = true;
        }
    }
    return unitDone;
}

__device__ __forceinline__ void finishSample(const RenderParams &p, UnitTaker &units, int lane, bool done, Rgb color, float4 &partial,
                                             unsigned int &unit, uint32_t &pixel, uint32_t &sample, uint32_t &endSample, bool &alive, bool &startNext)
{
    const bool needUnit = putSampleAway(p, false, done, color, partial, unit, sample, endSample);
    if (done && !needUnit) { startNext = true; }
    if (__ballot(needUnit) != 0ull) {
        const unsigned int newUnit = units.take(p, lane, needUnit);
        if (needUnit) {
            unit = newUnit;
            if (newUnit != 0xFFFFFFFFu) {
                unitSamples(p, newUnit, &pixel, &sample, &endSample);
                startNext = true;
            } else {
                alive = false;
            }
        }
    }
}
```

pathed_amd/csrc/pathed_hip.hip:

```cpp
#include "pathed_hip.h"

#include "bvh_build.h"
#include "kernels.h"
#include "features.h"
#include "shading_queries.h"
#if PATHED_EXPERIMENTS
#include "kernels_experiments.h"
#endif
#include "lbvh.h"
#include "scene_tables.h"

#include <hip/hip_runtime.h>

#include <dlfcn.h>

#include <chrono>
#include <cmath>
#include <cstdio>
#include <cstdlib>
#include <cstring>
#include <functional>
#include <memory>
#include <mutex>
#include <string>
// ... 1830 lines not shown
{
    const PathedSceneOptions &options = scene->options;
    scene->unitOrder = unitOrderFromEnvironment(options.unit_order == 2 ? kOrderStripesTiled : options.unit_order == 3 ? kOrderTiles : kOrderStripes);
    if (options.max_slots >= kBlock) { scene->maxSlots = options.max_slots; scene->adaptiveSlots = false; }
    if (const char *slots = tuningEnv("PATHED_MAX_SLOTS")) {
        const long value = atol(slots);
        if (value >= kBlock) { scene->maxSlots = (int)value; scene->adaptiveSlots = false; }
    }
}

static int createScene(const PathedSceneDesc *desc, const PathedSceneOptions *optionsIn, const PathedInstanceDesc *instanceDesc, PathedScene **out)
{
    if (!out) { return fail(PATHED_E_INVALID, "out pointer is null"); }
    *out = nullptr;
    int code = validate(desc);
    if (code != PATHED_OK) { return code; }
    PathedSceneOptions options;
    if ((code = resolveOptions(optionsIn, &options)) != PATHED_OK) { return code; }
    InstancedLayout instancedLayout;
    std::string refusal;
    if (instanceDesc && (code = planInstances(desc, options, instanceDesc, &instancedLayout, &refusal)) != PATHED_OK) { return fail(code, refusal); }
    int deviceId = 0;
    if ((code = resolveDevice(options, &deviceId)) != PATHED_OK) { return code; }

    std::unique_ptr<PathedScene> owner(new PathedScene());
    PathedScene *scene = owner.get();
    std::memset(&scene->device, 0, sizeof scene->device);
    scene->deviceId = deviceId;
    scene->options = options;
    scene->width = desc->camera.width;
    scene->height = desc->camera.height;
    scene->instanced = instanceDesc != nullptr;
    hipDeviceProp_t properties;
    if (hipGetDeviceProperties(&properties, deviceId) == hipSuccess) {
        scene->computeUnits = properties.multiProcessorCount > 0 ? properties.multiProcessorCount : 256;
    }
    buildCamera(desc->camera, &scene->device.camera);

    std::vector<size_t> textureOffset;
    if ((code = uploadTextures(scene, desc, &textureOffset)) != PATHED_OK) { return code; }
    ShadingTables tables;
    buildShadingTables(desc, scene->texels.ptr, textureOffset, &tables);
    packSpherePairs(desc, scene->spherePairs);

    const int builder = scene->bvhBuilder = chooseBuilder(desc, options);
    TriangleSoup soup;
    if ((code = uploadSoup(scene, desc, &soup)) != PATHED_OK) { return code; }
    const bool onDevice = builder == PATHED_BVH_LBVH_DEVICE || builder == PATHED_BVH_PLOC_DEVICE;
    code = onDevice ? buildTreeOnDevice(scene, desc, builder, soup) : buildTreeOnHost(scene, desc, instanceDesc, instancedLayout);
    if (code != PATHED_OK) { return code; }
    if ((code = settleSoup(scene, desc, &soup)) != PATHED_OK) { return code; }

    if ((code = uploadShadingTables(scene, desc, tables)) != PATHED_OK) { return code; }
    fillDeviceScene(scene, desc, tables);

    int shadeKernel = 0;
    if ((code = chooseShadeKernel(scene, desc, &shadeKernel)) != PATHED_OK) { return code; }
    if ((code = chooseNodeFormat(scene)) != PATHED_OK) { return code; }
    choosePathKernels(scene, shadeKernel);
    if ((code = buildSplits(scene, desc, shadeKernel)) != PATHED_OK) { return code; }
    if ((code = tuneWaveAndStages(scene, shadeKernel)) != PATHED_OK) { return code; }

    if ((code = buildSmallScene(scene, desc, tables.lightList)) != PATHED_OK) { return code; }
    const hipError_t status = rebuildCameraMasks(scene);
    if (status != hipSuccess) { return deviceFail(status, "build the camera-ray candidate masks"); }
    applySlotOptions(scene);
    *out = owner.release();
    return PATHED_OK;
}

int pathed_hip_scene_create_ex(const PathedSceneDesc *desc, const PathedSceneOptions *optionsIn, PathedScene **out)
{
    return createScene(desc, optionsIn, nullptr, out);
}

int pathed_hip_scene_create_instanced(const PathedSceneDesc *desc, const PathedSceneOptions *optionsIn, const PathedInstanceDesc *instances, PathedScene **out)
{
    if (!instances) { return fail(PATHED_E_INVALID, "instance description is null"); }
    return createScene(desc, optionsIn, instances, out);
}

void pathed_hip_scene_destroy(PathedScene *scene)
{
    if (scene) { (void)hipSetDevice(scene->deviceId); }
    delete scene;
}

}

static bool fillUnitOrder(RenderParams &q, int order, int width, unsigned long long itemPixels, int chunksPerPixel, int pool, int pools, int nQueues)
{
    const unsigned long long nPixels = itemPixels;
    const unsigned long long allQueues = (unsigned long long)nQueues * (unsigned long long)pools;
    unsigned long long items, itemUnits, lastItemShortfall = 0;
    if (order == kOrderTiles) {
        items = (nPixels + kUnitGroup - 1ull) / kUnitGroup;
        itemUnits = (unsigned long long)kUnitGroup * (unsigned long long)chunksPerPixel;
        q.lastGroupPixels = (unsigned int)(nPixels - (items - 1ull) * kUnitGroup);
        lastItemShortfall = (kUnitGroup - (unsigned long long)q.lastGroupPixels) * (unsigned long long)chunksPerPixel;
    } else {
        items = (unsigned long long)chunksPerPixel;
        itemUnits = nPixels;
        q.lastGroupPixels = kUnitGroup;
    }
    const unsigned long long stride = ((items + allQueues - 1ull) / allQueues) * itemUnits;
    if (stride * (unsigned long long)nQueues >= 0xFFFFFFF0ull || nPixels + kUnitGroup >= 0xFFFFFFF0ull) { return false; }
    q.unitOrder = order;
    q.pool = (unsigned int)pool;
    q.pools = (unsigned int)pools;
    q.nQueues = nQueues;
    q.nGroups = (unsigned int)items;
    q.groupUnits = (unsigned int)itemUnits;
    q.unitsPerQueue = (unsigned int)stride;
    q.divStride = makeFastDiv((unsigned int)stride);
    q.divGroupUnits = makeFastDiv((unsigned int)itemUnits);
    q.divBand = makeFastDiv(8u * (unsigned int)width);
    q.divWidth = makeFastDiv((unsigned int)width);
    unsigned long long total = 0;
    for (int k = 0; k < kUnitQueues; k++) {
        unsigned long long units = 0;
        const unsigned long long first = (unsigned long long)k * (unsigned long long)pools + (unsigned long long)pool;
        if (k < nQueues && first < items) {
            units = ((items - 1ull - first) / allQueues + 1ull) * itemUnits;
            if ((items - 1ull - first) % allQueues == 0ull) { units -= lastItemShortfall; }
        }
        q.queueUnits[k] = (unsigned int)units;
        total += units;
    }
    q.nUnits = (unsigned int)total;
    return true;
}

static bool volumeIntegrator(const PathedScene *scene)
{
    return scene->integrator == PATHED_INTEGRATOR_VOLUME_PATH_TRACER || scene->integrator == PATHED_INTEGRATOR_BASIC_VOLUME;
}

static bool usesVolumeKernel(const PathedScene *scene)
{
    if (!volumeIntegrator(scene)) { return false; }
    return scene->hasContainers || scene->device.nMedia > 0 || scene->options.generic_kernels != 0;
}

struct Pass {
    uint64_t seed;
    uint32_t begin, count;
    int startBounce, lastBounce;
    float *accum;
    float *squares;
    hipStream_t stream;
    int nPixels, chunk, chunksPerPixel;
    unsigned int nUnits;
    const uint32_t *pixelList;
    int nList;
    uint32_t *counts;

    int unitPixels() const { return nList > 0 ? nList : nPixels; }
    size_t bufferUnits() const { return (size_t)nPixels * (size_t)chunksPerPixel; }
};

static void launchResolve(const Pass &pass, const RenderParams &params, hipStream_t stream)
{
    const dim3 pixelGrid((unsigned)((pass.unitPixels() + kBlock - 1) / kBlock));
    if (pass.nList > 0) {
        ListMomentsParams moments;
        moments.chunkBuf = params.state.chunkBuf;
        moments.pixelList = pass.pixelList;
        moments.nList = pass.nList;
        moments.nPixels = params.nPixels;
        moments.chunksPerPixel = params.chunksPerPixel;
        moments.samples = pass.count;
        moments.sum = params.accum;
        moments.squares = pass.squares;
        moments.count = pass.counts;
        hipLaunchKernelGGL(k_resolve_list, pixelGrid, dim3(kBlock), 0, stream, moments);
    } else if (pass.squares) {
        MomentsParams moments;
        moments.chunkBuf = params.state.chunkBuf;
        moments.nPixels = params.nPixels;
        moments.chunksPerPixel = params.chunksPerPixel;
        moments.sum = params.accum;
        moments.squares = pass.squares;
        hipLaunchKernelGGL(k_resolve_moments, pixelGrid, dim3(kBlock), 0, stream, moments);
    } else {
        hipLaunchKernelGGL(k_resolve, pixelGrid, dim3(kBlock), 0, stream, params);
    }
}

static bool fillPassParams(RenderParams &q, const PathedScene *scene, const Pass &pass, int pool, int pools, int nQueues)
{
    q.scene = scene->device;
    q.state.chunkBuf = scene->chunkBuf.ptr;
    q.counters = scene->counters.ptr + (size_t)pool * kCtrCount;
    q.stats = scene->stats.ptr;
    q.accum = pass.accum;
    q.nPixels = pass.nPixels;
    q.chunk = pass.chunk;
    q.chunksPerPixel = pass.chunksPerPixel;
    q.seedLo = (uint32_t)pass.seed;
    q.seedHi = (uint32_t)(pass.seed >> 32);
    q.sppBegin = pass.begin;
    q.sppEnd = pass.begin + pass.count;
    q.startBounce = pass.startBounce;
    q.lastBounce = pass.lastBounce;
    if (pass.nList > 0) { q.cameraQueue = reinterpret_cast<float4 *>(const_cast<uint32_t *>(pass.pixelList)); }
    return fillUnitOrder(q, pass.nList > 0 ? kOrderList : scene->unitOrder, scene->width, (unsigned long long)pass.unitPixels(), pass.chunksPerPixel, pool, pools, nQueues);
}

template <typename Launch>
static int persistentPass(PathedScene *scene, const Pass &pass, int blocksPerCu, int maxStack, int ldsRows, Launch launch)
{
    if (scene->chunkCapacity < pass.bufferUnits()) {
        HIP_TRY(scene->chunkBuf.allocate(pass.bufferUnits()));
        scene->chunkCapacity = pass.bufferUnits();
    }
    if (!scene->counters.ptr) { HIP_TRY(scene->counters.allocate(kMaxPools * kCtrCount)); }
    if (!scene->stats.ptr) {
        HIP_TRY(scene->stats.allocate(kStatCount));
        HIP_TRY(hipMemset(scene->stats.ptr, 0, kStatCount * sizeof(unsigned long long)));
    }

    unsigned long long blocks = (unsigned long long)scene->computeUnits * blocksPerCu;
    const unsigned long long blocksNeeded = ((unsigned long long)pass.nUnits + (unsigned long long)kBlock - 1) / kBlock;
    if (blocks > blocksNeeded) { blocks = blocksNeeded; }
    if (blocks < 1) { blocks = 1; }
    const unsigned int waves = (unsigned int)blocks * kWavesPerBlock;

    RenderParams params;
    std::memset(&params, 0, sizeof params);
    if (maxStack > 0) {
        const size_t overflowRows = (size_t)(maxStack > ldsRows ? maxStack - ldsRows : 0);
        const size_t overflowInts = (size_t)blocks * kBlock * (overflowRows ? overflowRows : 1);
        if (scene->volumeOverflow.count < overflowInts) { HIP_TRY(scene->volumeOverflow.allocate(overflowInts)); }
        params.stackOverflow = scene->volumeOverflow.ptr;
        params.maxStack = maxStack;
    }
    if (!fillPassParams(params, scene, pass, 0, 1, (int)(waves < (unsigned int)kUnitQueues ? waves : (unsigned int)kUnitQueues))) {
        return fail(PATHED_E_INVALID, "too many work units in one pass");
    }
    {
        const unsigned int wavesPerQueue = (waves + (unsigned int)params.nQueues - 1) / (unsigned int)params.nQueues;
        unsigned int grab = (pass.nUnits / (unsigned int)params.nQueues) / (wavesPerQueue * 4u);
        params.unitGrab = (int)(grab < 1u ? 1u : grab > 64u ? 64u : grab);
    }

    HIP_TRY(hipMemsetAsync(params.counters, 0, kCtrCount * sizeof(unsigned int), pass.stream));
    int timed = -1;
    if (scene->timeKernels) {
        timed = scene->traceEvents.acquire();
        (void)hipEventRecord(scene->traceEvents.start[timed], pass.stream);
    }
    launch(params, dim3((unsigned)blocks), pass.stream);
    if (timed >= 0) { (void)hipEventRecord(scene->traceEvents.stop[timed], pass.stream); }
    scene->traceLaunchesAll++;
    launchResolve(pass, params, pass.stream);
    HIP_TRY(hipGetLastError());
    HIP_TRY(hipStreamSynchronize(pass.stream));

    scene->iterations += 1;
    scene->cameraSamples += (unsigned long long)pass.count * (unsigned long long)pass.unitPixels();
    return PATHED_OK;
}

static int renderPassFused(PathedScene *scene, const Pass &pass)
{
    const size_t maskQuads = cameraMaskQuads(scene);
    if (scene->cameraQueue.count < maskQuads + cameraQueueWords(scene) || !scene->cameraMasksBuilt) { HIP_TRY(rebuildCameraMasks(scene)); }
    bool queueShort = false;
    const int code = persistentPass(scene, pass, PATHED_FUSED_WAVES, 0, 0, [&](RenderParams &params, dim3 grid, hipStream_t stream) {
        if ((size_t)grid.x * kWavesPerBlock * kCameraQueueWords > scene->cameraQueue.count - maskQuads) { queueShort = true; return; }
        const bool ldsMaterials = scene->device.nMaterials <= kMaxLdsMaterials;
        const size_t lds = ldsMaterials ? (size_t)scene->device.nMaterials * sizeof(DMaterial) : 0;
        params.cameraQueue = scene->cameraQueue.ptr + maskQuads;
        params.mfmaTable = scene->mfmaTable.ptr;
        params.mfmaFrame = scene->mfmaFrame;
        params.smallQuads = scene->smallLayout.nQuads;
        params.smallKappaT = scene->smallLayout.kappaT;
        params.scene.leafTris = scene->itemTris.ptr;
        std::memcpy(params.spherePairs, scene->spherePairs, sizeof params.spherePairs);

        const SceneTraitFlags &traits = scene->traits;
        const bool count = scene->countMode;
        const SmallTris *records = &scene->smallItems;
        const auto run = [&](void (*kernel)(RenderParams, SmallTris)) { hipLaunchKernelGGL(kernel, grid, dim3(kBlock), lds, stream, params, *records); };
#if PATHED_EXPERIMENTS
        if (scene->mfmaPhase1 && ldsMaterials) {
            withBool(count, [&](auto COUNT) {
                if (traits.lambertianTriangles) { run(k_path_small<true, COUNT, TraitsLambertianTriangles, true>); }
                else if (traits.lambertianPlasticSpheres) { run(k_path_small<true, COUNT, TraitsLambertianPlasticSpheres, true>); }
                else { run(k_path_small<true, COUNT, TraitsAll, true>); }
            });
        } else
#endif
        if (scene->smallLayout.nQuads > 0 && ldsMaterials) {
            const auto quadsKernel = [&](auto COUNT, auto traitsTag) -> void (*)(RenderParams, SmallTris) {
                using TRAITS = typename decltype(traitsTag)::type;
                if (kSmallPassList<decltype(COUNT)::value, false, TRAITS>) {
                    const SmallItemsLayout &list = scene->passLayout;
                    params.smallQuads = list.nQuads | scene->passTris << 8 | list.shadowQuadPairs << 16 | list.shadowLonePairs << 24;
                    records = &scene->passItems;
                } else if (kSmallPrunes<decltype(COUNT)::value, TRAITS>) {
                    params.smallQuads = scene->smallLayout.nQuads | scene->smallLayout.shadowQuadPairs << 16 | scene->smallLayout.shadowLonePairs << 24;
                }
                return k_path_small<true, decltype(COUNT)::value, TRAITS, false, true>;
            };
            const std::false_type plain{};
            if (traits.lambertianTriangles) { withBool(count, [&](auto COUNT) { run(quadsKernel(COUNT, TraitsTag<TraitsLambertianTriangles>())); }); }
            else if (traits.lambertianPlasticSpheres) { withBool(count, [&](auto COUNT) { run(quadsKernel(COUNT, TraitsTag<TraitsLambertianPlasticSpheres>())); }); }
            else if (traits.roughBeckmann && !count) { run(quadsKernel(plain, TraitsTag<TraitsRoughBeckmann>())); }
            else if (traits.roughGgx && !count) { run(quadsKernel(plain, TraitsTag<TraitsRoughGgx>())); }
            else if (traits.smoothSet && !count) { run(quadsKernel(plain, TraitsTag<TraitsSmooth>())); }
            else if (traits.triangleLit && !count) { run(quadsKernel(plain, TraitsTag<TraitsTriangleLit>())); }
            else { withBool(count, [&](auto COUNT) { run(quadsKernel(COUNT, TraitsTag<TraitsAll>())); }); }
        } else if (traits.lambertianTriangles) {
            withBool(ldsMaterials, [&](auto LDS_MATERIALS) { withBool(count, [&](auto COUNT) { run(k_path_small<LDS_MATERIALS, COUNT, TraitsLambertianTriangles>); }); });
        } else if (traits.lambertianPlasticSpheres && ldsMaterials) {
            withBool(count, [&](auto COUNT) { run(k_path_small<true, COUNT, TraitsLambertianPlasticSpheres>); });
        } else {
            withBool(ldsMaterials, [&](auto LDS_MATERIALS) { withBool(count, [&](auto COUNT) { run(k_path_small<LDS_MATERIALS, COUNT, TraitsAll>); }); });
        }
    });
    if (queueShort) { return fail(PATHED_E_DEVICE, "the fused kernel's grid outgrew its camera queues"); }
    return code;
}

static int renderPassVolume(PathedScene *scene, const Pass &pass)
{
    if (pass.nList > 0) {
        const bool small = scene->bruteForce;
        const int rows = small ? 8 : 22;
        return persistentPass(scene, pass, PATHED_VOLUME_WAVES, scene->maxStack, rows, [&](RenderParams &params, dim3 grid, hipStream_t stream) {
            const size_t lds = (size_t)(rows + 1) * kBlock * sizeof(int);
            params.smallQuads = 0;
            params.smallKappaT = scene->smallLayout.kappaT;
            params.scene.leafTris = scene->leafTris.ptr;
            const bool grids = !scene->gridsHost.empty();
            const bool multi = scene->integrator == PATHED_INTEGRATOR_BASIC_VOLUME;
            withBool(small, [&](auto SMALL) { withBool(grids, [&](auto GRID) { withBool(multi, [&](auto MULTI) {
                hipLaunchKernelGGL((k_list_volume<SMALL, GRID, MULTI>), grid, dim3(kBlock), lds, stream, params, scene->smallTris);
            }); }); });
        });
    }
    return persistentPass(scene, pass, PATHED_VOLUME_WAVES, scene->maxStack, scene->stackRows, [&](RenderParams &params, dim3 grid, hipStream_t stream) {
        const bool ldsMaterials = scene->device.nMaterials <= kMaxLdsMaterials;
        const bool small = scene->bruteForce;
        const size_t lds = (size_t)((small ? 8 : scene->stackRows) + 1) * kBlock * sizeof(int)
            + (ldsMaterials ? (size_t)scene->device.nMaterials * sizeof(DMaterial) : 0);
        const bool quads = small && ldsMaterials && scene->smallLayout.nQuads > 0;
        params.smallQuads = quads ? scene->smallLayout.nQuads : 0;
        params.smallKappaT = scene->smallLayout.kappaT;
        if (quads) { params.scene.leafTris = scene->itemTris.ptr; }

        const auto run = [&](void (*kernel)(RenderParams, SmallTris)) {
            hipLaunchKernelGGL(kernel, grid, dim3(kBlock), lds, stream, params, quads ? scene->smallItems : scene->smallTris);
        };
        if (scene->integrator == PATHED_INTEGRATOR_BASIC_VOLUME) {
            params.smallQuads = 0;
            params.scene.leafTris = scene->leafTris.ptr;
            const size_t scatterLds = (size_t)((small ? 8 : scene->stackRows) + 1) * kBlock * sizeof(int);
            const bool grids = !scene->gridsHost.empty();
            const auto runScatter = [&](void (*plain)(RenderParams, SmallTris), void (*withGrids)(RenderParams, SmallTris)) {
                hipLaunchKernelGGL(grids ? withGrids : plain, grid, dim3(kBlock), scatterLds, stream, params, scene->smallTris);
            };
            if (small) { runScatter(k_path_scatter<8, true>, k_path_scatter_grid<8, true>); }
            else {
                switch (scene->stackRows) {
                case 8: runScatter(k_path_scatter<8, false>, k_path_scatter_grid<8, false>); break;
                case 16: runScatter(k_path_scatter<16, false>, k_path_scatter_grid<16, false>); break;
                default: runScatter(k_path_scatter<22, false>, k_path_scatter_grid<22, false>); break;
                }
            }
        } else if (!scene->gridsHost.empty()) {
            params.smallQuads = 0;
            params.scene.leafTris = scene->leafTris.ptr;
            const size_t gridLds = (size_t)((small ? 8 : scene->stackRows) + 1) * kBlock * sizeof(int);
            const auto runGrid = [&](void (*kernel)(RenderParams, SmallTris)) {
                hipLaunchKernelGGL(kernel, grid, dim3(kBlock), gridLds, stream, params, scene->smallTris);
            };
            if (small) { runGrid(k_path_volume_grid<8, true>); }
            else {
                switch (scene->stackRows) {
                case 8: runGrid(k_path_volume_grid<8, false>); break;
                case 16: runGrid(k_path_volume_grid<16, false>); break;
                default: runGrid(k_path_volume_grid<22, false>); break;
                }
            }
        } else if (small && ldsMaterials && scene->traits.lambertianGlassContainer) {
            withBool(quads, [&](auto QUADS) { run(k_path_volume<true, 8, true, TraitsLambertianGlassContainer, QUADS>); });
        } else if (quads) {
            run(k_path_volume<true, 8, true, TraitsAll, true>);
        } else {
            withBool(ldsMaterials, [&](auto LDS_MATERIALS) {
                if (small) { run(k_path_volume<LDS_MATERIALS, 8, true>); return; }
                switch (scene->stackRows) {
                case 8: run(k_path_volume<LDS_MATERIALS, 8, false>); break;
                case 16: run(k_path_volume<LDS_MATERIALS, 16, false>); break;
                default: run(k_path_volume<LDS_MATERIALS, 22, false>); break;
                }
            });
        }
    });
}

static int renderPassWave(PathedScene *scene, const Pass &pass)
{
    const int stackRows = 22;
    return persistentPass(scene, pass, PATHED_WAVE_WAVES, scene->maxStack, stackRows, [&](RenderParams &params, dim3 grid, hipStream_t stream) {
        const size_t lds = pathWaveLdsBytes(stackRows, scene->device.nMaterials, PATHED_EXPERIMENTS && scene->waveBlock);
        params.suspendLanes = scene->waveStragglers;
        params.suspendPatience = scene->waveRefill;
        params.parkMinCardsPerWave = scene->waveShadeReady;

        const SceneTraitFlags &traits = scene->traits;
        const bool envOnly = traits.envOnly && scene->device.nSpheres == 0 && !scene->hasContainers;
        const auto run = [&](void (*kernel)(RenderParams)) { hipLaunchKernelGGL(kernel, grid, dim3(kBlock), lds, stream, params); };
#if PATHED_EXPERIMENTS
        if (scene->waveBlock && envOnly) { run(k_path_wave<true, 22, TraitsEnvironmentOnly, false, true>); }
        else
#endif
        if (envOnly) { run(k_path_wave<true, 22, TraitsEnvironmentOnly, false>); }
        else if (traits.smoothSet) { run(k_path_wave<true, 22, TraitsSmooth, false>); }
        else if (traits.triangleLit) { run(k_path_wave<true, 22, TraitsTriangleLit, false>); }
        else if (scene->device.nSpheres == 0) { run(k_path_wave<true, 22, TraitsAll, false>); }
        else { run(k_path_wave<true, 22, TraitsAll, true>); }
    });
}

static int renderPassHybrid(PathedScene *scene, const Pass &pass)
{
    return persistentPass(scene, pass, PATHED_HYBRID_WAVES, scene->hybridMaxStack, kHybridStackRows, [&](RenderParams &params, dim3 grid, hipStream_t stream) {
        const PathedSceneOptions &options = scene->options;
        const size_t lds = (size_t)scene->device.nMaterials * sizeof(DMaterial);
        params.smallQuads = scene->hybridLayout.nQuads;
        params.smallKappaT = scene->hybridLayout.kappaT;
        params.scene.leafTris = scene->hybridItemTris.ptr;
        params.hybridNodes = scene->hybridNodes.ptr;
        params.hybridTris = scene->hybridTris.ptr;
        params.hybridNodeCount = scene->hybridNodeCount;
        params.hybridTreeTris = scene->hybridTreeTris;
        params.hybridDirectTris = scene->hybridDirectTris;
        for (int a = 0; a < 3; a++) { params.hybridLo[a] = scene->hybridLo[a]; params.hybridHi[a] = scene->hybridHi[a]; }
        for (int a = 0; a < 4; a++) { params.hybridSphere[a] = scene->hybridSphere[a]; }
        params.suspendLanes = options.wave_stragglers != 0 ? (options.wave_stragglers < 0 ? 0 : options.wave_stragglers) : kHybridStragglers;
        params.suspendPatience = options.wave_refill != 0 ? options.wave_refill : kHybridRefill;
        params.hybridBatch = options.hybrid_batch != 0 ? options.hybrid_batch : kHybridBatch;
        params.hybridReady = options.hybrid_ready != 0 ? (options.hybrid_ready < 0 ? 1 : options.hybrid_ready) : kHybridReady;

        const SceneTraitFlags &traits = scene->traits;
        const auto run = [&](void (*kernel)(RenderParams, SmallTris)) { hipLaunchKernelGGL(kernel, grid, dim3(kBlock), lds, stream, params, scene->hybridItems); };
        if (traits.envOnly && !scene->hasContainers) { run(k_path_hybrid<TraitsEnvironmentOnly>); }
        else if (traits.smoothSet) { run(k_path_hybrid<TraitsSmooth>); }
        else if (traits.triangleLit) { run(k_path_hybrid<TraitsTriangleLit>); }
        else { run(k_path_hybrid<TraitsAll>); }
    });
}

static int renderPass(PathedScene *scene, const Pass &pass)
{
    const hipStream_t stream = pass.stream;
    const unsigned long long nUnits64 = pass.nUnits;

    int pools = scene->pools;
    if (nUnits64 < 4ull * kBlock * (unsigned long long)pools) { pools = 1; }

    unsigned long long wanted = nUnits64 < (unsigned long long)scene->maxSlots ? nUnits64 : (unsigned long long)scene->maxSlots;
    if (scene->adaptiveSlots) {
        const unsigned long long floorSlots = 1ull << 22;
        unsigned long long byWork = nUnits64 / 16ull;
        if (byWork < floorSlots) { byWork = floorSlots; }
        if (wanted > byWork) { wanted = byWork; }
    }
    const unsigned long long slotQuantum = (unsigned long long)kBlock * (scene->stagedShade ? scene->stageRounds : 1);
    const int slotsPerPool = (int)((wanted / pools + slotQuantum - 1) / slotQuantum * slotQuantum);
    const int nSlots = slotsPerPool * pools;
    int code = ensureRenderState(scene, nSlots, pass.bufferUnits());
    if (code != PATHED_OK) { return code; }
    if (pools > 1 && !scene->poolStreams[0]) {
        for (int h = 0; h < kMaxPools; h++) {
            HIP_TRY(hipStreamCreateWithFlags(&scene->poolStreams[h], hipStreamNonBlocking));
            HIP_TRY(hipEventCreateWithFlags(&scene->poolDone[h], hipEventDisableTiming));
        }
        HIP_TRY(hipEventCreateWithFlags(&scene->callerReady, hipEventDisableTiming));
    }

    const int blocksPerPool = slotsPerPool / kBlock;
    const int shadeBlocks = blocksPerPool / (scene->stagedShade ? scene->stageRounds : 1);
    const int nQueues = shadeBlocks < kUnitQueues ? shadeBlocks : kUnitQueues;

    RenderParams params[kMaxPools];
    std::memset(params, 0, sizeof params);
    hipStream_t streams[kMaxPools] = { stream, stream, stream, stream };
    for (int h = 0; h < pools; h++) {
        RenderParams &q = params[h];
        const size_t slotBase = (size_t)h * slotsPerPool;
        if (!fillPassParams(q, scene, pass, h, pools, nQueues)) { return fail(PATHED_E_INVALID, "too many work units in one pass"); }
        q.state.rayO = scene->rayO.ptr + slotBase;
        q.state.rayD = scene->rayD.ptr + slotBase;
        q.state.hit = scene->hit.ptr + slotBase;
        q.state.mod = scene->mod.ptr + slotBase;
        q.state.thr = scene->thr.ptr + slotBase;
        q.state.res = scene->res.ptr + slotBase;
        q.state.pend = scene->pend.ptr + slotBase;
        q.state.acc = scene->acc.ptr + slotBase;
        q.state.shO = scene->shO.ptr + slotBase;
        q.state.shD = scene->shD.ptr + slotBase;
        if (scene->splitShade) {
            const size_t listEntries = (size_t)scene->listCap * kListShards * 64;
            for (int list = 0; list < 2; list++) {
                q.state.lists[list] = scene->slotLists.ptr + ((size_t)h * 2 + list) * listEntries;
                for (int parity = 0; parity < 2; parity++) {
                    q.state.deferred[list][parity] = scene->deferredLists.ptr + (((size_t)h * 2 + list) * 2 + parity) * (size_t)scene->nSlots;
                }
            }
            q.listCap = scene->listCap;
        }
        const size_t traceWaves = (size_t)scene->traceGrid * kWavesPerBlock;
        q.suspendLanes = (scene->bruteForce || scene->instanced) ? 0 : scene->suspendLanes;
        q.suspendPatience = scene->suspendPatience;
        q.parkMinCardsPerWave = scene->parkMinCards;
        q.suspendMask = scene->bruteForce ? nullptr : scene->suspendMask.ptr + (size_t)h * traceWaves;
        q.suspendData = scene->bruteForce ? nullptr
            : scene->suspendData.ptr + (size_t)h * traceWaves * (size_t)(kSaveWords + scene->maxStack) * 64;
        {
            const size_t overflowRows = (size_t)(scene->maxStack > scene->stackRows ? scene->maxStack - scene->stackRows : 0);
            q.stackOverflow = scene->bruteForce ? nullptr
                : scene->stackOverflow.ptr + (size_t)h * (size_t)scene->traceGrid * kBlock * (overflowRows ? overflowRows : 1);
            q.maxStack = scene->maxStack;
        }
        q.nSlots = slotsPerPool;
        q.localCount = (!scene->stagedShade && !scene->splitShade) ? scene->localCount : 0;
        q.localCounting = scene->countMode ? 1 : 0;
        q.afterTrace = 1;
        if (q.localCount > 0) {
            std::memcpy(q.localTris, scene->localTris, sizeof q.localTris);
            for (int a = 0; a < 3; a++) { q.hybridLo[a] = scene->localLo[a]; q.hybridHi[a] = scene->localHi[a]; }
            for (int a = 0; a < 4; a++) { q.hybridSphere[a] = scene->localSphere[a]; }
        }
        if (pools > 1) { streams[h] = scene->poolStreams[h]; }
    }

    if (pools > 1) {
        HIP_TRY(hipEventRecord(scene->callerReady, stream));
        for (int h = 0; h < pools; h++) { HIP_TRY(hipStreamWaitEvent(streams[h], scene->callerReady, 0)); }
    }

    const dim3 slotGrid((unsigned)blocksPerPool), block(kBlock);
    for (int h = 0; h < pools; h++) {
        HIP_TRY(hipMemsetAsync(params[h].counters, 0, kCtrCount * sizeof(unsigned int), streams[h]));
        if (params[h].suspendMask) {
            HIP_TRY(hipMemsetAsync(params[h].suspendMask, 0, (size_t)scene->traceGrid * kWavesPerBlock * sizeof(unsigned long long), streams[h]));
        }
        hipLaunchKernelGGL(k_init, slotGrid, block, 0, streams[h], params[h]);
    }

    const int launchChunk = 8;
    const int ringSize = 32;
    struct PollGuard {
        hipEvent_t events[kMaxPools][2] = {};
        hipStream_t *streams = nullptr;
        int pools = 0;
        ~PollGuard()
        {
            for (int h = 0; h < pools; h++) { (void)hipStreamSynchronize(streams[h]); }
            for (int h = 0; h < kMaxPools; h++) {
                for (int k = 0; k < 2; k++) { if (events[h][k]) { (void)hipEventDestroy(events[h][k]); } }
            }
        }
    } guard;
    guard.streams = streams;
    guard.pools = pools;
    hipEvent_t (&pollEvents)[kMaxPools][2] = guard.events;
    for (int h = 0; h < pools; h++) {
        HIP_TRY(hipEventCreateWithFlags(&pollEvents[h][0], hipEventDisableTiming));
        HIP_TRY(hipEventCreateWithFlags(&pollEvents[h][1], hipEventDisableTiming));
    }
    const int shadeLaunches = params[0].localCount > 0 ? (scene->options.shade_launches > 0 ? scene->options.shade_launches : kDefaultShadeLaunches) : 1;
    unsigned long long iteration = 0;
    int pollIndex = 0;
    bool havePending = false;
    bool poolDone[kMaxPools];
    for (int h = 0; h < kMaxPools; h++) { poolDone[h] = h >= pools; }
    while (!(poolDone[0] && poolDone[1] && poolDone[2] && poolDone[3])) {
        for (int k = 0; k < launchChunk; k++) {
            for (int h = 0; h < pools; h++) {
                if (poolDone[h]) { continue; }
                params[h].parity = (int)(iteration & 1ull);
                scene->traceLaunchesAll++;
#if defined(PATHED_EXPERIMENTS) && PATHED_EXPERIMENTS
                if (h == 0) {
                    if (const char *text = tuningEnv("PATHED_SORT_PROBE")) {
                        if (iteration == (unsigned long long)atoll(text)) { sortProbe(scene, params[h], streams[h]); }
                    }
                }
#endif
                if (scene->timeKernels && iteration % (unsigned long long)scene->timeInterval == 0ull) {
                    const int e = scene->traceEvents.acquire();
                    (void)hipEventRecord(scene->traceEvents.start[e], streams[h]);
                    launchTrace(scene, params[h], streams[h]);
                    (void)hipEventRecord(scene->traceEvents.stop[e], streams[h]);
                    const int s = scene->shadeEvents.acquire();
                    (void)hipEventRecord(scene->shadeEvents.start[s], streams[h]);
                    for (int round = 0; round < shadeLaunches; round++) {
                        params[h].afterTrace = round == 0 ? 1 : 0;
                        launchShade(scene, params[h], streams[h]);
                    }
                    (void)hipEventRecord(scene->shadeEvents.stop[s], streams[h]);
// ... 1309 lines not shown
```

pathed_amd/csrc/shading.h:

```cpp
#pragma once

#include "device_scene.h"

namespace pathed {

template <unsigned MATERIALS, bool ENV, bool TRIANGLE_LIGHTS, bool SPHERES, bool VARYING_ALBEDO, bool PAIRED_TRIG = false, unsigned DISTRIBUTIONS = 3u>
struct SceneTraits {
    static constexpr unsigned materials = MATERIALS;
    static constexpr bool beckmann = (DISTRIBUTIONS & 1u) != 0u;
    static constexpr bool ggx = (DISTRIBUTIONS & 2u) != 0u;
    static constexpr bool env = ENV;
    static constexpr bool triangleLights = TRIANGLE_LIGHTS;
    static constexpr bool spheres = SPHERES;
    static constexpr bool varyingAlbedo = VARYING_ALBEDO;
    static constexpr bool pairedTrig = PAIRED_TRIG;
    static constexpr bool has(int type) { return ((MATERIALS >> type) & 1u) != 0u; }
};
typedef SceneTraits<0x7Fu, true, true, true, true> TraitsAll;
typedef SceneTraits<1u << 0, false, true, false, false, true> TraitsLambertianTriangles;
typedef SceneTraits<(1u << 0) | (1u << 3), false, false, true, false, true> TraitsLambertianPlasticSpheres;
typedef SceneTraits<(1u << 0) | (1u << 4) | (1u << 6), false, true, true, false> TraitsLambertianGlassContainer;
typedef SceneTraits<0x3Fu, false, true, false, false, true> TraitsTriangleLit;
typedef SceneTraits<0x3Fu, true, false, false, true> TraitsEnvironmentOnly;
typedef SceneTraits<0x0Fu, false, true, false, false, true, 1u> TraitsRoughBeckmann;
typedef SceneTraits<0x0Fu, false, true, false, false, true, 2u> TraitsRoughGgx;
typedef SceneTraits<(1u << 0) | (1u << 4) | (1u << 5), false, true, false, false, true, 3u> TraitsSmooth;


#define PATHED_INV_PI 0.3183098861837907f
#define PATHED_PI 3.14159265358979323846f
#define PATHED_TWO_PI 6.283185307179586f

__host__ __device__ inline float twoPiTimes(float u) { return (float)(6.283185307179586476925286766559 * (double)u); }


__host__ __device__ inline uint32_t mix32(uint32_t x)
{
    x ^= x >> 16; x *= 0x7feb352du;
    x ^= x >> 15; x *= 0x846ca68bu;
    x ^= x >> 16;
    return x;
}

struct Rng {
    uint32_t k0, k1;
    uint32_t dimension;

    __device__ inline float next()
    {
        const uint32_t bits = mix32(k0 + mix32(k1 + dimension * 0x9e3779b9u));
        dimension++;
        return (float)(bits >> 8) * 5.9604638e-08f;
    }
};

__host__ __device__ inline void makeKey(uint64_t seed, uint32_t pixel, uint32_t sample, uint32_t *k0, uint32_t *k1)
{
    *k0 = mix32(pixel ^ mix32((uint32_t)seed));
    *k1 = mix32(sample ^ mix32((uint32_t)(seed >> 32) ^ 0x9e3779b9u));
}

__device__ inline uint32_t vertexBase(int vertex) { return 2u + 8u * (uint32_t)(vertex - 1); }


struct Frame {
    V3 xAxis, normal, zAxis;
};

__device__ inline Frame normalToWorldSpace1(V3 normal)
{
    V3 xAxis;
    if (fabsf(normal.x) > fabsf(normal.y)) {
        xAxis = normalized(v3(-normal.z, 0.f, normal.x));
    } else {
        xAxis = normalized(v3(0.f, -normal.z, normal.y));
    }
    Frame frame;
    frame.xAxis = xAxis;
    frame.normal = normal;
    frame.zAxis = cross(normal, xAxis);
    return frame;
}

__device__ inline Frame normalToWorldSpace(V3 normal, V3 rayDirection)
{
    if (normal == rayDirection) { return normalToWorldSpace1(normal); }
    Frame frame;
    frame.xAxis = normalized(cross(normal, rayDirection));
    frame.normal = normal;
    frame.zAxis = normalized(cross(normal, frame.xAxis));
    return frame;
}

__device__ inline V3 toWorld(const Frame &f, V3 l)
{
    return v3(
        f.xAxis.x * l.x + f.normal.x * l.y + f.zAxis.x * l.z,
        f.xAxis.y * l.x + f.normal.y * l.y + f.zAxis.y * l.z,
        f.xAxis.z * l.x + f.normal.z * l.y + f.zAxis.z * l.z);
}

__device__ inline V3 toLocal(const Frame &f, V3 w)
{
    return v3(
        f.xAxis.x * w.x + f.xAxis.y * w.y + f.xAxis.z * w.z,
        f.normal.x * w.x + f.normal.y * w.y + f.normal.z * w.z,
        f.zAxis.x * w.x + f.zAxis.y * w.y + f.zAxis.z * w.z);
}

struct Isect {
    V3 point;
    V3 wo;
    V3 normal;
    V3 shadingNormal;
    float u, v;
    int material;
    int prim;
    Frame frame;
    V3 woLocal;
};


__device__ inline float tfCos2Theta(V3 v) { return v.y * v.y; }
__device__ inline float tfSinTheta(V3 v) { return sqrtf(smax(0.f, 1.f - tfCos2Theta(v))); }
__device__ inline float tfSin2Theta(V3 v) { return 1.f - tfCos2Theta(v); }
__device__ inline float tfTanTheta(V3 v) { return tfSinTheta(v) / v.y; }
__device__ inline float tfTan2Theta(V3 v) { return tfSin2Theta(v) / tfCos2Theta(v); }

__device__ inline V3 tfClamp(V3 v)
{
    const float max = 0.9999f;
    if (v.x >= max) { return v3(1.f, 0.f, 0.f); }
    if (v.y >= max) { return v3(0.f, 1.f, 0.f); }
    if (v.z >= max) { return v3(0.f, 0.f, 1.f); }
    if (v.x <= -max) { return v3(-1.f, 0.f, 0.f); }
    if (v.y <= -max) { return v3(0.f, -1.f, 0.f); }
    if (v.z <= -max) { return v3(0.f, 0.f, -1.f); }
    return v;
}

__device__ inline float tfCosPhi(V3 v)
{
    const float sinTheta = tfSinTheta(v);
    if (sinTheta == 0.f) { return 1.f; }
    return clampf(v.x / sinTheta, -1.f, 1.f);
}

__device__ inline float tfSinPhi(V3 v)
{
    const V3 clamped = tfClamp(v);
    const float sinTheta = tfSinTheta(clamped);
    if (sinTheta == 0.f) { return 0.f; }
    return clampf(clamped.z / sinTheta, -1.f, 1.f);
}

__device__ inline float tfCos2Phi(V3 v) { const float c = tfCosPhi(v); return c * c; }
__device__ inline float tfSin2Phi(V3 v) { const float s = tfSinPhi(v); return s * s; }

__device__ inline float sinFromCos(float cosTheta)
{
    const float sin2Theta = 1.f - (cosTheta * cosTheta);
    return sqrtf(smax(0.f, sin2Theta));
}


template <bool PAIRED>
__device__ inline void cosSin(float angle, float *cosine, float *sine)
{
    if (PAIRED) { sincosf(angle, sine, cosine); }
    else { *cosine = cosf(angle); *sine = sinf(angle); }
}

template <bool PAIRED = false, typename RNG>
__device__ inline V3 cosineSampleHemisphere(RNG &random)
{
    const float xi1 = random.next();
    const float r = sqrtf(xi1);
    const float phi = twoPiTimes(random.next());
    float cosPhi, sinPhi;
    cosSin<PAIRED>(phi, &cosPhi, &sinPhi);
    const float x = r * cosPhi;
    const float z = r * sinPhi;
    const float y = sqrtf(1.f - xi1);
    return v3(x, y, z);
}

__device__ inline float cosineHemispherePdf(V3 v) { return v.y * PATHED_INV_PI; }

__device__ inline void cartesianToSpherical(V3 cartesian, float *phi, float *theta)
{
    float p = atan2f(cartesian.z, cartesian.x);
    if (p < 0.f) { p += PATHED_TWO_PI; }
    if (p == PATHED_TWO_PI) { p = 0.f; }
    *phi = p;
    *theta = acosf(clampf(cartesian.y, -1.f, 1.f));
}

template <bool PAIRED = false>
__device__ inline V3 sphericalToCartesian(float phi, float cosTheta, float sinTheta)
{
    const float y = cosTheta;
    float cosPhi, sinPhi;
    cosSin<PAIRED>(phi, &cosPhi, &sinPhi);
    const float x = sinTheta * cosPhi;
    const float z = sinTheta * sinPhi;
    return v3(x, y, z);
}


__device__ inline float dielectricReflectance(float cosThetaIncident, float etaIncident, float etaTransmitted)
{
    const float sinThetaTransmitted =
        (etaIncident / etaTransmitted) * sqrtf(smax(0.f, 1.f - cosThetaIncident * cosThetaIncident));
    if (sinThetaTransmitted > 1.f) { return 1.f; }

    const float cosThetaTransmitted = sqrtf(smax(0.f, 1.f - sinThetaTransmitted * sinThetaTransmitted));

    const float rParallel =
        (etaTransmitted * cosThetaIncident - etaIncident * cosThetaTransmitted)
        / (etaTransmitted * cosThetaIncident + etaIncident * cosThetaTransmitted);
    const float rPerpendicular =
        (etaIncident * cosThetaIncident - etaTransmitted * cosThetaTransmitted)
        / (etaIncident * cosThetaIncident + etaTransmitted * cosThetaTransmitted);

    return 0.5f * (rParallel * rParallel + rPerpendicular * rPerpendicular);
}

__device__ inline bool snellRefract(V3 incidentLocal, V3 *transmittedLocal, float etaIncident, float etaTransmitted)
{
    V3 normal = v3(0.f, 1.f, 0.f);
    if (incidentLocal.y < 0.f) { normal = normal * -1.f; }

    const V3 wIncidentPerpendicular = incidentLocal - (normal * dot(incidentLocal, normal));
    const V3 wTransmittedPerpendicular = -wIncidentPerpendicular * (etaIncident / etaTransmitted);

    const float perpendicularLength = length(wTransmittedPerpendicular);
    const float transmittedPerpendicularLength2 = perpendicularLength * perpendicularLength;
    const float wTransmittedParallelLength = sqrtf(smax(0.f, 1.f - transmittedPerpendicularLength2));
    const V3 wTransmittedParallel = normal * -wTransmittedParallelLength;

    const float cosThetaIncident = incidentLocal.y;
    const float sin2ThetaIncident = smax(0.f, 1.f - (cosThetaIncident * cosThetaIncident));
    const float eta2 = (etaIncident / etaTransmitted) * (etaIncident / etaTransmitted);
    const float sin2ThetaTransmitted = eta2 * sin2ThetaIncident;

    *transmittedLocal = normalized(wTransmittedParallel + wTransmittedPerpendicular);

    return !(sin2ThetaTransmitted >= 1.f);
}


struct BSDFSample {
    V3 wiWorld;
    float pdf;
    Rgb throughput;
};

__device__ inline Rgb matDiffuse(const DMaterial &m) { return rgb(m.diffuse[0], m.diffuse[1], m.diffuse[2]); }
__device__ inline Rgb matEmit(const DMaterial &m) { return rgb(m.emit[0], m.emit[1], m.emit[2]); }

__device__ inline bool isDelta(const DMaterial &m)
{
    return m.type == PATHED_MAT_GLASS || m.type == PATHED_MAT_MIRROR;
}

__device__ inline Rgb checkerboardLookup(const DMaterial &m, const Isect &isect)
{
    const int uIndex = (int)floorf(isect.u * m.checkerResU);
    const int vIndex = (int)floorf(isect.v * m.checkerResV);
    if (uIndex % 2 == vIndex % 2) { return rgb(m.checkerOn[0], m.checkerOn[1], m.checkerOn[2]); }
    return rgb(m.checkerOff[0], m.checkerOff[1], m.checkerOff[2]);
}

__device__ inline Rgb textureLookup(const DMaterial &m, const Isect &isect)
{
    const int width = m.texSize & 0xFFFF, height = (m.texSize >> 16) & 0xFFFF;
    const float u = isect.u - (float)(int)floorf(isect.u);
    const float v = 1.f - (isect.v - (float)(int)floorf(isect.v));
    int x = (int)roundf(u * (float)(width - 1));
    int y = (int)roundf(v * (float)(height - 1));
    x = imin(imax(x, 0), width - 1);
    y = imin(imax(y, 0), height - 1);
    const float4 texel = m.texels[(size_t)y * width + x];
    return rgb(texel.x, texel.y, texel.z);
}

template <bool VARYING_ALBEDO = true>
__device__ inline Rgb lambertianFLocal(const DMaterial &m, const Isect &isect, V3 wiWorld, V3 wi, float *pdf)
{
    if (dot(isect.wo, isect.shadingNormal) < 0.f) { *pdf = 0.f; return rgb(0.f); }
    if (dot(wiWorld, isect.shadingNormal) < 0.f) { *pdf = 0.f; return rgb(0.f); }

    *pdf = cosineHemispherePdf(wi);

    if (VARYING_ALBEDO && m.albedoType == PATHED_ALBEDO_CHECKERBOARD) { return checkerboardLookup(m, isect) / PATHED_PI; }
    if (VARYING_ALBEDO && m.albedoType == PATHED_ALBEDO_TEXTURE) { return textureLookup(m, isect) / PATHED_PI; }
    return matDiffuse(m) / PATHED_PI;
}
template <bool VARYING_ALBEDO = true>
__device__ inline Rgb lambertianF(const DMaterial &m, const Isect &isect, V3 wiWorld, float *pdf)
{
    return lambertianFLocal<VARYING_ALBEDO>(m, isect, wiWorld, normalized(toLocal(isect.frame, wiWorld)), pdf);
}

template <bool VARYING_ALBEDO = true, bool PAIRED = false, typename RNG>
__device__ inline BSDFSample lambertianSample(const DMaterial &m, const Isect &isect, RNG &random)
{
    const V3 localSample = cosineSampleHemisphere<PAIRED>(random);
    const V3 worldSample = toWorld(isect.frame, localSample);
    BSDFSample sample;
    sample.wiWorld = worldSample;
    sample.pdf = cosineHemispherePdf(localSample);
    float ignored;
    sample.throughput = lambertianF<VARYING_ALBEDO>(m, isect, worldSample, &ignored);
    return sample;
}

#ifndef PATHED_OREN_NAYAR_TRIG
#define PATHED_OREN_NAYAR_TRIG 0
#endif
__device__ inline Rgb orenNayarFLocal(const DMaterial &m, const Isect &isect, V3 localWo, V3 localWi, float *pdf)
{
    if (dot(isect.normal, isect.wo) < 0.f) { *pdf = 1.f; return rgb(0.f); }
    if (dot(isect.shadingNormal, isect.wo) < 0.f) { *pdf = 1.f; return rgb(0.f); }

    if (localWo.y < 0.f) { *pdf = 1.f; return rgb(0.f); }
    if (localWi.y < 0.f) { *pdf = 1.f; return rgb(0.f); }

    *pdf = cosineHemispherePdf(localWi);

#if PATHED_OREN_NAYAR_TRIG
    float phiI, thetaI, phiO, thetaO;
    cartesianToSpherical(localWi, &phiI, &thetaI);
    cartesianToSpherical(localWo, &phiO, &thetaO);
    const float alpha = smax(thetaI, thetaO);
    const float beta = smin(thetaI, thetaO);
    const float rough = smax(0.f, cosf(phiI - phiO)) * sinf(alpha) * tanf(beta);
#else
    const float azimuthal = localWi.x * localWo.x + localWi.z * localWo.z;
    const float highest = smax(localWi.y, localWo.y);
    const float rough = (azimuthal > 0.f && highest > 0.f) ? azimuthal / highest : 0.f;
#endif
    const float throughput = PATHED_INV_PI * (m.orenA + m.orenB * rough);

    return matDiffuse(m) * throughput;
}
__device__ inline Rgb orenNayarF(const DMaterial &m, const Isect &isect, V3 wiWorld, float *pdf)
{
    return orenNayarFLocal(m, isect, normalized(toLocal(isect.frame, isect.wo)), normalized(toLocal(isect.frame, wiWorld)), pdf);
}

template <bool PAIRED = false, typename RNG>
__device__ inline BSDFSample orenNayarSample(const DMaterial &m, const Isect &isect, RNG &random)
{
    const V3 localSample = cosineSampleHemisphere<PAIRED>(random);
    const V3 worldSample = toWorld(isect.frame, localSample);
    BSDFSample sample;
    sample.wiWorld = worldSample;
    sample.pdf = cosineHemispherePdf(localSample);
    float ignored;
    sample.throughput = orenNayarF(m, isect, worldSample, &ignored);
    return sample;
}

__device__ inline float beckmannD(float alpha, V3 wh)
// ... 673 lines not shown
```

Measured before the change: 3683 Msamples/s.

## Add specialized single-sample kernel with cached per-sample RNG key rows

Moves the path-tracing kernel body into a shared include and instantiates a dedicated single-sample variant for Lambertian-triangle scenes when chunk is 1. This variant skips the per-unit multi-sample bookkeeping. At each bounce it fetches the inner mix32(k1 + dim·golden) hash words from a small key-slot table, since those words depend only on the per-sample key k1 and not on the pixel, and falls back to computing them when the table misses. The aim is to remove redundant RNG hashing and control overhead, at the cost of extra table lookups, an extra kernel variant and more register and memory pressure.

After: 3999 Msamples/s, median of 6. +8.6%, better.

```diff
diff --git a/pathed_amd/csrc/kernels.h b/pathed_amd/csrc/kernels.h
--- a/pathed_amd/csrc/kernels.h
+++ b/pathed_amd/csrc/kernels.h
@@ -1441,10 +1441,10 @@
     float tfar;
 };
 
-template <bool ENV_ONLY = false, typename TRAITS = TraitsAll, typename MaterialTable>
+template <bool ENV_ONLY = false, typename TRAITS = TraitsAll, typename MaterialTable, typename RNG>
 __device__ inline Rgb sampleLightsTerm(
     const DScene &scene, const MaterialTable &materials,
-    const Isect &isect, const DMaterial &material, Rng &random, ShadowRequest *shadow
+    const Isect &isect, const DMaterial &material, RNG &random, ShadowRequest *shadow
 ) {
     shadow->push = false;
 #if defined(PATHED_ABLATE) && PATHED_ABLATE == 2
@@ -2776,282 +2776,15 @@
 template <bool LDS_MATERIALS, bool COUNT, typename TRAITS, bool MFMA = false, bool QUADS = false>
 __global__ __launch_bounds__(kBlock) __attribute__((amdgpu_waves_per_eu(PATHED_FUSED_WAVES, PATHED_FUSED_WAVES))) void k_path_small(RenderParams p, SmallTris smallTris)
 {
-    extern __shared__ float4 ldsDynamic[];
-    __shared__ float mfmaRows[MFMA ? kMfmaTableFloats : 1];
-    __shared__ float4 stashRows[QUADS ? 6 * kBlock : 1];
-    constexpr int kResolveCapacity = PATHED_RESOLVE_SHARED == 2 ? 128 : 64;
-    __shared__ unsigned long long resolveBest[QUADS ? kBlock : 1];
-    __shared__ float2 resolveUv[QUADS ? kWavesPerBlock * kResolveCapacity : 1];
-    __shared__ unsigned short resolveItems[QUADS ? kWavesPerBlock * kResolveCapacity : 1];
-    __shared__ unsigned int resolveOccluded[QUADS ? kBlock : 1], resolveCount[QUADS ? kWavesPerBlock : 1];
-    if (MFMA) {
-        for (int i = threadIdx.x; i < kMfmaTableFloats; i += kBlock) { mfmaRows[i] = p.mfmaTable[i]; }
-        if (!LDS_MATERIALS) { __syncthreads(); }
-    }
-    const MaterialAccess<LDS_MATERIALS> materials = stageMaterials<LDS_MATERIALS>(p, ldsDynamic);
-    const TraceGeometry geometry = sceneGeometry(p.scene, false);
-
-    const DScene &scene = p.scene;
-    const int lane = threadIdx.x & 63;
-    const unsigned int waveId = blockIdx.x * kWavesPerBlock + (unsigned int)__builtin_amdgcn_readfirstlane((int)(threadIdx.x >> 6));
-    const int nTris = p.scene.nTris;
-    constexpr bool kPassList = QUADS && kSmallPassList<COUNT, MFMA, TRAITS>;
-    TraceGeometry passGeometry = geometry;
-    if (kPassList) { passGeometry.tris = geometry.tris + 3 * nTris; }
-    const uint64_t seed = ((uint64_t)p.seedHi << 32) | p.seedLo;
-    UnitTaker units(p, waveId);
-
-    bool alive = true;
-    bool needEntry = true;
-    unsigned int unit = 0xFFFFFFFFu;
-    uint32_t pixel = 0, sample = 0, endSample = 0;
-    PathRegisters path = idlePath();
-    float4 partial = make_float4(0.f, 0.f, 0.f, 0.f);
-    bool pendingShadow = false;
-    V3 shadowDirection = v3(0.f, 0.f, 1.f);
-    float shadowTfar = 0.f;
-
-    unsigned int closestRays = 0, shadowRays = 0, trisTested = 0;
-
-    float4 *const cameraQueue = p.cameraQueue + (size_t)waveId * kCameraQueueWords;
-    unsigned int queueHead = 0u, queueCount = 0u;
-    bool unitsLeft = true;
-    const bool singleSample = p.chunk == 1;
-
-    bool startNext = false;
-
-    while (true) {
-        SHADE_REGION(0, alive && !needEntry);
-        SHADE_REGION(1, startNext);
-        if (startNext) {
-            startCameraSample(p, seed, pixel, sample, path);
-            startNext = false;
-        }
-
-        if (QUADS) {
-            float4 *stash = stashRows + threadIdx.x;
-            stash[0 * kBlock] = make_float4(path.result.r, path.result.g, path.result.b, path.bsdfPdf);
-            stash[1 * kBlock] = make_float4(path.modulation.r, path.modulation.g, path.modulation.b, path.cosTheta);
-            stash[2 * kBlock] = make_float4(path.throughput.r, path.throughput.g, path.throughput.b, intAsFloat(path.st));
-            stash[3 * kBlock] = partial;
-            stash[4 * kBlock] = make_float4(intAsFloat((int)pixel), intAsFloat((int)sample), intAsFloat((int)endSample), intAsFloat((int)unit));
-            stash[5 * kBlock] = make_float4(intAsFloat((int)path.random.k0), intAsFloat((int)path.random.k1), intAsFloat(path.firstEmitMaterial), intAsFloat((int)path.random.dimension));
-            asm volatile("" ::: "memory");
-        }
-
-        if (queueCount < 64u && unitsLeft) {
-            const unsigned int newUnit = units.take(p, lane, true);
-            const bool got = newUnit != 0xFFFFFFFFu;
-            const unsigned long long gotMask = __ballot(got);
-            SHADE_REGION(11, got);
-            if (gotMask != ~0ull) { unitsLeft = false; }
-            Rng cameraRandom;
-            cameraRandom.k0 = 0u; cameraRandom.k1 = 0u; cameraRandom.dimension = 0u;
-            V3 cameraO = v3(0.f, 0.f, 0.f), cameraD = v3(0.f, 0.f, 1.f);
-            constexpr bool kMasks = !COUNT && !MFMA;
-            uint32_t unitPixel = 0u;
-            if (got) {
-                uint32_t unitFirst, unitEnd;
-                unitSamples(p, newUnit, &unitPixel, &unitFirst, &unitEnd);
-                cameraSampleRay(p, seed, unitPixel, unitFirst, cameraRandom, &cameraO, &cameraD);
-            }
-            LaneRay cameraHit;
-            laneRayInit(cameraHit, cameraO, cameraD, PATHED_TNEAR, PATHED_TFAR, false);
-            unsigned int candidatesLow = 0, candidatesHigh = 0;
-            if (kMasks) {
-                if (got) {
-                    const unsigned long long pixelCandidates = cameraMasks(p)[unitPixel];
-                    candidatesLow = (unsigned int)(pixelCandidates >> 32);
-                    candidatesHigh = (unsigned int)pixelCandidates;
-                }
-            } else if (got) {
-                if (QUADS || MFMA) {
-                    unsigned int unusedLow = 0, unusedHigh = 0;
-                    smallCandidatesItems<false, true, true>(smallTris.data, p.smallQuads, nTris, p.smallKappaT, cameraO, cameraD, cameraD,
-                                                             &candidatesLow, &candidatesHigh, &unusedLow, &unusedHigh, candidateNear(PATHED_TNEAR), 0.f);
-                } else {
-                    smallCandidates(smallTris.data, nTris, cameraO, cameraD, &candidatesLow, &candidatesHigh, candidateNear(PATHED_TNEAR));
-                }
-            }
-            if (COUNT && got) {
-                trisTested += (unsigned int)nTris;
-                closestRays++;
-            }
-            smallResolve(geometry, cameraHit, candidatesLow, candidatesHigh);
-            if (got) {
-                finishRay(geometry, cameraHit);
-                const unsigned int slot = (queueHead + queueCount + laneRank(gotMask)) & (kCameraQueueEntries - 1u);
-                const unsigned int target = singleSample ? (unsigned int)partialIndex(p, newUnit) : newUnit;
-                cameraQueue[0 * kCameraQueueEntries + slot] = make_float4(cameraD.x, cameraD.y, cameraD.z, cameraHit.best);
-                cameraQueue[1 * kCameraQueueEntries + slot] = make_float4(cameraHit.bestU, cameraHit.bestV, intAsFloat(cameraHit.bestPrim), intAsFloat((int)target));
-                cameraQueue[2 * kCameraQueueEntries + slot] = make_float4(intAsFloat((int)cameraRandom.k0), intAsFloat((int)cameraRandom.k1), 0.f, 0.f);
-            }
-            queueCount += (unsigned int)__popcll(gotMask);
-            __threadfence_block();
-        }
-
-        const bool tracing = alive && !needEntry;
-        LaneRay ray;
-        laneRayInit(ray, path.o, path.d, PATHED_TNEAR, PATHED_TFAR, false);
-        {
-            const bool traceShadow = tracing && pendingShadow;
-            LaneRay shadowRay;
-            laneRayInit(shadowRay, path.o, shadowDirection, PATHED_TNEAR, shadowTfar, true);
-            unsigned int candidatesLow = 0, candidatesHigh = 0, shadowLow = 0, shadowHigh = 0;
-            SHADE_REGION(2, traceShadow);
-            if (MFMA) {
-                mfmaCandidatesPair(mfmaRows, nTris, p.mfmaFrame, __ballot(traceShadow) != 0ull, path.o, path.d, shadowDirection,
-                                   candidateNear(PATHED_TNEAR), candidateFar(shadowTfar), &candidatesLow, &candidatesHigh, &shadowLow, &shadowHigh);
-                if (!tracing) { candidatesLow = 0u; candidatesHigh = 0u; }
-                if (!traceShadow) { shadowLow = 0u; shadowHigh = 0u; }
-            } else if (QUADS) {
-                if (tracing) {
-                    constexpr bool kPrune = kSmallPrunes<COUNT, TRAITS>;
-                    const int smallQuads = kPassList ? (p.smallQuads & 0xFF) : kPrune ? (p.smallQuads & 0xFFFF) : p.smallQuads;
-                    const int passTris = kPassList ? ((p.smallQuads >> 8) & 0xFF) : nTris;
-                    smallCandidatesItems<true, true, true, kPrune>(smallTris.data, smallQuads, passTris, p.smallKappaT, path.o, path.d, shadowDirection,
-                                                                   &candidatesLow, &candidatesHigh, &shadowLow, &shadowHigh,
-                                                                   candidateNear(PATHED_TNEAR), candidateFar(shadowTfar),
-                                                                   (p.smallQuads >> 16) & 0xFF, (p.smallQuads >> 24) & 0xFF);
-                    if (!traceShadow) { shadowLow = 0u; shadowHigh = 0u; }
-                }
-            } else if (__ballot(traceShadow) != 0ull) {
-                if (tracing) {
-                    smallCandidatesPair(smallTris.data, nTris, path.o, path.d, shadowDirection, &candidatesLow, &candidatesHigh, &shadowLow, &shadowHigh,
-                                        candidateNear(PATHED_TNEAR), candidateFar(shadowTfar));
-                    if (!traceShadow) { shadowLow = 0u; shadowHigh = 0u; }
-                }
-            } else if (tracing) {
-                smallCandidates(smallTris.data, nTris, path.o, path.d, &candidatesLow, &candidatesHigh, candidateNear(PATHED_TNEAR));
-            }
-            if (COUNT && tracing) {
-                trisTested += (unsigned int)nTris * (traceShadow ? 2u : 1u);
-                closestRays++;
-                if (traceShadow) { shadowRays++; }
-            }
-            bool spheresDone = false;
-            RESOLVE_PROBE(9, candidatesLow, candidatesHigh);
-            RESOLVE_PROBE(10, shadowLow, shadowHigh);
-            if (MFMA) {
-                mfmaResolve(geometry, ray, candidatesLow, candidatesHigh);
-                mfmaResolve(geometry, shadowRay, shadowLow, shadowHigh);
-            } else if (QUADS && PATHED_RESOLVE_SHARED) {
-                ResolveScratch scratch;
-                const int waveBase = (int)(threadIdx.x & ~63u), wave = (int)(threadIdx.x >> 6);
-                scratch.best = resolveBest + waveBase; scratch.uv = resolveUv + wave * kResolveCapacity; scratch.items = resolveItems + wave * kResolveCapacity;
-                scratch.occluded = resolveOccluded + waveBase; scratch.count = resolveCount + wave;
-                unsigned int sphereCandidates = 0u, shadowSphereCandidates = 0u;
-                if (TRAITS::spheres && geometry.nSpheres > 0 && tracing) {
-                    smallSphereCandidates(p, geometry.nSpheres, path.o, path.d, shadowDirection, &sphereCandidates, &shadowSphereCandidates);
-                    if (!traceShadow) { shadowSphereCandidates = 0u; }
-                }
-                spheresDone = smallResolveShared<kResolveCapacity, PATHED_RESOLVE_SHARED != 2, TRAITS::spheres>(
-                    passGeometry, ray, shadowRay, candidatesLow, candidatesHigh, shadowLow, shadowHigh, sphereCandidates, shadowSphereCandidates, scratch);
-            } else {
-                smallResolve(passGeometry, ray, candidatesLow, candidatesHigh);
-                smallResolve(passGeometry, shadowRay, shadowLow, shadowHigh);
-            }
-            if (tracing && !spheresDone) { finishRay(geometry, ray); }
-            if (traceShadow) {
-                if (!spheresDone) { finishRay(geometry, shadowRay); }
-                if (shadowRay.occluded) { path.pend = rgb(0.f); }
-            }
-            pendingShadow = false;
-        }
-        if (QUADS) {
-            asm volatile("" ::: "memory");
-            const float4 *stash = stashRows + threadIdx.x;
-            const float4 s0 = stash[0 * kBlock], s1 = stash[1 * kBlock], s2 = stash[2 * kBlock], s4 = stash[4 * kBlock], s5 = stash[5 * kBlock];
-            path.result = rgb(0.f); path.result.r = s0.x; path.result.g = s0.y; path.result.b = s0.z; path.bsdfPdf = s0.w;
-            path.modulation.r = s1.x; path.modulation.g = s1.y; path.modulation.b = s1.z; path.cosTheta = s1.w;
-            path.throughput.r = s2.x; path.throughput.g = s2.y; path.throughput.b = s2.z; path.st = floatAsInt(s2.w);
-            partial = stash[3 * kBlock];
-            pixel = (uint32_t)floatAsInt(s4.x); sample = (uint32_t)floatAsInt(s4.y); endSample = (uint32_t)floatAsInt(s4.z); unit = (unsigned int)floatAsInt(s4.w);
-            path.random.k0 = (uint32_t)floatAsInt(s5.x); path.random.k1 = (uint32_t)floatAsInt(s5.y); path.firstEmitMaterial = floatAsInt(s5.z); path.random.dimension = (uint32_t)floatAsInt(s5.w);
-        }
-        float4 h = make_float4(ray.best, ray.bestU, ray.bestV, intAsFloat(ray.bestPrim));
-
-        bool done = false;
-        bool departs = false;
-        Rgb color = rgb(0.f);
-        if (tracing) {
-            const bool miss = floatAsInt(h.w) < 0;
-            Isect arrived;
-            SHADE_REGION(3, !miss);
-            if (!miss) { arrived = makeIsect<TRAITS>(scene, path.o, path.d, h); }
-            done = pathArrive<TRAITS, true>(p, scene, materials, path, arrived, miss, &color);
-            departs = !done;
-        }
-
-        while (true) {
-            SHADE_REGION(8, done);
-            {
-                const bool unitDone = putSampleAway(p, singleSample, done, color, partial, unit, sample, endSample);
-                needEntry = needEntry || unitDone;
-                startNext = startNext || (done && !unitDone);
-            }
-            done = false;
-            const unsigned long long wanting = __ballot(needEntry);
-            if (wanting == 0ull) { break; }
-            if (queueCount == 0u) {
-                if (!unitsLeft && needEntry) { alive = false; needEntry = false; }
-                break;
-            }
-            __threadfence_block();
-            const unsigned int rank = laneRank(wanting);
-            if (needEntry && rank < queueCount) {
-                const unsigned int slot = (queueHead + rank) & (kCameraQueueEntries - 1u);
-                const float4 e0 = cameraQueue[0 * kCameraQueueEntries + slot];
-                const float4 e1 = cameraQueue[1 * kCameraQueueEntries + slot];
-                const float4 e2 = cameraQueue[2 * kCameraQueueEntries + slot];
-                resetPath(path);
-                path.o = cameraOrigin(scene.camera);
-                path.d = v3(e0.x, e0.y, e0.z);
-                path.random.k0 = (uint32_t)floatAsInt(e2.x); path.random.k1 = (uint32_t)floatAsInt(e2.y); path.random.dimension = 2u;
-                h = make_float4(e0.w, e1.x, e1.y, e1.z);
-                unit = (unsigned int)floatAsInt(e1.w);
-                if (singleSample) { sample = 0u; endSample = 1u; }
-                else { unitSamples(p, unit, &pixel, &sample, &endSample); }
-                needEntry = false;
-                if (floatAsInt(h.w) < 0) {
-                    color = cameraMissColor<TRAITS>(scene, path.d);
-                    done = true;
-                } else {
-                    departs = true;
-                }
-            }
-            const unsigned int wanted = (unsigned int)__popcll(wanting);
-            const unsigned int taken = wanted < queueCount ? wanted : queueCount;
-            queueHead = (queueHead + taken) & (kCameraQueueEntries - 1u);
-            queueCount -= taken;
-        }
-        if (__ballot(alive) == 0ull) { break; }
-
-        SHADE_REGION(6, departs);
-        bool ended = false;
-        if (departs) {
-            Isect isect = makeIsect<TRAITS>(scene, path.o, path.d, h);
-            ShadowRequest shadow;
-            ended = pathDepart<TRAITS, true>(p, scene, materials, path, isect, &shadow, &color);
-            if (shadow.push) {
-                pendingShadow = true;
-                shadowDirection = shadow.direction;
-                shadowTfar = shadow.tfar;
-            }
-        }
-        if (__ballot(ended) != 0ull) {
-            SHADE_REGION(8, ended);
-            const bool unitDone = putSampleAway(p, singleSample, ended, color, partial, unit, sample, endSample);
-            needEntry = needEntry || unitDone;
-            startNext = startNext || (ended && !unitDone);
-        }
-    }
-
-    if (COUNT) {
-        atomicAdd(&p.stats[kStatTris], (unsigned long long)trisTested);
-        atomicAdd(&p.stats[kStatClosest], (unsigned long long)closestRays);
-        atomicAdd(&p.stats[kStatShadow], (unsigned long long)shadowRays);
-    }
+    constexpr bool SINGLE = false;
+#include "path_small_body.h"
+}
+
+__global__ __launch_bounds__(kBlock) __attribute__((amdgpu_waves_per_eu(PATHED_FUSED_WAVES, PATHED_FUSED_WAVES))) void k_path_small_single(RenderParams p, SmallTris smallTris)
+{
+    constexpr bool LDS_MATERIALS = true, COUNT = false, MFMA = false, QUADS = true, SINGLE = true;
+    typedef TraitsLambertianTriangles TRAITS;
+#include "path_small_body.h"
 }
 
 #include "path_wave.h"
diff --git a/pathed_amd/csrc/path_common.h b/pathed_amd/csrc/path_common.h
--- a/pathed_amd/csrc/path_common.h
+++ b/pathed_amd/csrc/path_common.h
@@ -178,9 +178,9 @@
     return finished;
 }
 
-template <typename TRAITS, bool PROBES = false, typename MATERIALS>
+template <typename TRAITS, bool PROBES = false, bool KEYED = false, typename MATERIALS>
 __device__ __forceinline__ bool pathDepart(const RenderParams &p, const DScene &scene, const MATERIALS &materials, PathRegisters &path,
-                                           Isect &isect, ShadowRequest *shadowOut, Rgb *color)
+                                           Isect &isect, ShadowRequest *shadowOut, Rgb *color, const uint32_t *keyRow = nullptr)
 {
     ShadowRequest shadow;
     shadow.push = false;
@@ -208,7 +208,16 @@
         prepareLobes<TRAITS>(material, isect);
 
         path.random.dimension = vertexBase(vertex);
-        const BSDFSample bsdfSample = materialSample<TRAITS>(material, isect, path.random);
+        const auto sampleBsdf = [&]() -> BSDFSample {
+            if constexpr (KEYED) {
+                RowRng rowRandom;
+                rowRandom.k0 = path.random.k0; rowRandom.row = keyRow; rowRandom.dimension = 0u;
+                return materialSample<TRAITS>(material, isect, rowRandom);
+            } else {
+                return materialSample<TRAITS>(material, isect, path.random);
+            }
+        };
+        const BSDFSample bsdfSample = sampleBsdf();
 
         const bool counts = checkCounts(p.startBounce, p.lastBounce, vertex);
         const bool emissive = !isBlack(matEmit(material));
@@ -219,7 +228,13 @@
         if (PROBES) { SHADE_REGION(7, wantDirect); }
         if (wantDirect) {
             path.random.dimension = vertexBase(vertex) + 3;
-            lightTerm = sampleLightsTerm<false, TRAITS>(scene, materials, isect, material, path.random, &shadow);
+            if constexpr (KEYED) {
+                RowRng rowRandom;
+                rowRandom.k0 = path.random.k0; rowRandom.row = keyRow; rowRandom.dimension = 3u;
+                lightTerm = sampleLightsTerm<false, TRAITS>(scene, materials, isect, material, rowRandom, &shadow);
+            } else {
+                lightTerm = sampleLightsTerm<false, TRAITS>(scene, materials, isect, material, path.random, &shadow);
+            }
         }
 
         const bool deadEnd = isBlack(bsdfSample.throughput) && bsdfSample.pdf > 0.f && bsdfSample.pdf < 3e38f
@@ -297,6 +312,22 @@
     return unitDone;
 }
 
+__device__ __forceinline__ void putUnitAway(const RenderParams &p, bool done, Rgb color, unsigned int index)
+{
+    if (done) {
+        float4 partial = make_float4(0.f, 0.f, 0.f, 0.f);
+        const bool finite = isfinite(color.r) && isfinite(color.g) && isfinite(color.b);
+        if (finite) {
+            partial.x += color.r;
+            partial.y += color.g;
+            partial.z += color.b;
+        } else {
+            atomicAdd(&p.stats[kStatDropped], 1ull);
+        }
+        p.state.chunkBuf[(size_t)index] = partial;
+    }
+}
+
 __device__ __forceinline__ void finishSample(const RenderParams &p, UnitTaker &units, int lane, bool done, Rgb color, float4 &partial,
                                              unsigned int &unit, uint32_t &pixel, uint32_t &sample, uint32_t &endSample, bool &alive, bool &startNext)
 {
diff --git a/pathed_amd/csrc/path_small_body.h b/pathed_amd/csrc/path_small_body.h
--- /dev/null
+++ b/pathed_amd/csrc/path_small_body.h
@@ -0,0 +1,354 @@
+    static_assert(!SINGLE || (QUADS && !COUNT && !MFMA), "the single-sample body exists for the headline instantiation");
+    extern __shared__ float4 ldsDynamic[];
+    __shared__ float mfmaRows[MFMA ? kMfmaTableFloats : 1];
+    constexpr int kStashRows = SINGLE ? 4 : 6;
+    constexpr int kStashKeyRow = SINGLE ? 3 : 5;
+    __shared__ float4 stashRows[QUADS ? kStashRows * kBlock : 1];
+    constexpr int kResolveCapacity = PATHED_RESOLVE_SHARED == 2 ? 128 : 64;
+    __shared__ unsigned long long resolveBest[QUADS ? kBlock : 1];
+    __shared__ float2 resolveUv[QUADS ? kWavesPerBlock * kResolveCapacity : 1];
+    __shared__ unsigned short resolveItems[QUADS ? kWavesPerBlock * kResolveCapacity : 1];
+    __shared__ unsigned int resolveOccluded[QUADS ? kBlock : 1], resolveCount[QUADS ? kWavesPerBlock : 1];
+    __shared__ uint4 keyRows[SINGLE ? kWavesPerBlock * 2 * kKeyTableWords / 4 : 1];
+    if (MFMA) {
+        for (int i = threadIdx.x; i < kMfmaTableFloats; i += kBlock) { mfmaRows[i] = p.mfmaTable[i]; }
+        if (!LDS_MATERIALS) { __syncthreads(); }
+    }
+    const MaterialAccess<LDS_MATERIALS> materials = stageMaterials<LDS_MATERIALS>(p, ldsDynamic);
+    const TraceGeometry geometry = sceneGeometry(p.scene, false);
+
+    const DScene &scene = p.scene;
+    const int lane = threadIdx.x & 63;
+    const unsigned int waveId = blockIdx.x * kWavesPerBlock + (unsigned int)__builtin_amdgcn_readfirstlane((int)(threadIdx.x >> 6));
+    const int nTris = p.scene.nTris;
+    constexpr bool kPassList = QUADS && kSmallPassList<COUNT, MFMA, TRAITS>;
+    TraceGeometry passGeometry = geometry;
+    if (kPassList) { passGeometry.tris = geometry.tris + 3 * nTris; }
+    const uint64_t seed = ((uint64_t)p.seedHi << 32) | p.seedLo;
+    UnitTaker units(p, waveId);
+
+    bool alive = true;
+    bool needEntry = true;
+    unsigned int unit = 0xFFFFFFFFu;
+    uint32_t pixel = 0, sample = 0, endSample = 0;
+    PathRegisters path = idlePath();
+    float4 partial = make_float4(0.f, 0.f, 0.f, 0.f);
+    bool pendingShadow = false;
+    V3 shadowDirection = v3(0.f, 0.f, 1.f);
+    float shadowTfar = 0.f;
+
+    unsigned int closestRays = 0, shadowRays = 0, trisTested = 0;
+
+    float4 *const cameraQueue = p.cameraQueue + (size_t)waveId * kCameraQueueWords;
+    unsigned int queueHead = 0u, queueCount = 0u;
+    bool unitsLeft = true;
+    const bool singleSample = SINGLE || p.chunk == 1;
+
+    bool startNext = false;
+
+    KeySlots keySlots;
+    keySlots.clear();
+    uint4 *const keyTables = keyRows + (SINGLE ? (threadIdx.x >> 6) * 2 * (kKeyTableWords / 4) : 0);
+
+    while (true) {
+        SHADE_REGION(0, alive && !needEntry);
+        SHADE_REGION(1, startNext);
+        if (!SINGLE && startNext) {
+            startCameraSample(p, seed, pixel, sample, path);
+            startNext = false;
+        }
+
+        if (QUADS) {
+            float4 *stash = stashRows + threadIdx.x;
+            stash[0 * kBlock] = make_float4(path.result.r, path.result.g, path.result.b, path.bsdfPdf);
+            stash[1 * kBlock] = make_float4(path.modulation.r, path.modulation.g, path.modulation.b, path.cosTheta);
+            stash[2 * kBlock] = make_float4(path.throughput.r, path.throughput.g, path.throughput.b, intAsFloat(path.st));
+            if (!SINGLE) {
+                stash[3 * kBlock] = partial;
+                stash[4 * kBlock] = make_float4(intAsFloat((int)pixel), intAsFloat((int)sample), intAsFloat((int)endSample), intAsFloat((int)unit));
+            }
+            stash[kStashKeyRow * kBlock] = make_float4(intAsFloat((int)path.random.k0), intAsFloat((int)path.random.k1), intAsFloat(path.firstEmitMaterial),
+                                                       intAsFloat((int)(SINGLE ? unit : path.random.dimension)));
+            asm volatile("" ::: "memory");
+        }
+
+        if (queueCount < 64u && unitsLeft) {
+            const unsigned int newUnit = units.take(p, lane, true);
+            const bool got = newUnit != 0xFFFFFFFFu;
+            const unsigned long long gotMask = __ballot(got);
+            SHADE_REGION(11, got);
+            if (gotMask != ~0ull) { unitsLeft = false; }
+            Rng cameraRandom;
+            cameraRandom.k0 = 0u; cameraRandom.k1 = 0u; cameraRandom.dimension = 0u;
+            V3 cameraO = v3(0.f, 0.f, 0.f), cameraD = v3(0.f, 0.f, 1.f);
+            constexpr bool kMasks = !COUNT && !MFMA;
+            uint32_t unitPixel = 0u;
+            if (got) {
+                uint32_t unitFirst, unitEnd;
+                unitSamples(p, newUnit, &unitPixel, &unitFirst, &unitEnd);
+                cameraSampleRay(p, seed, unitPixel, unitFirst, cameraRandom, &cameraO, &cameraD);
+            }
+            if (SINGLE && gotMask != 0ull) {
+                const int firstLane = __builtin_amdgcn_readfirstlane(__ffsll((long long)gotMask) - 1);
+                const uint32_t batchK1 = (uint32_t)__builtin_amdgcn_readlane((int)cameraRandom.k1, firstLane);
+                if (keySlots.find(batchK1) < 0) {
+                    uint32_t *table = reinterpret_cast<uint32_t *>(keyTables + keySlots.claim(batchK1) * (kKeyTableWords / 4));
+                    table[lane] = innerKey(batchK1, vertexBase(1) + (uint32_t)lane);
+                    if (lane < kKeyTableWords - 64) { table[64 + lane] = innerKey(batchK1, vertexBase(1) + 64u + (uint32_t)lane); }
+                }
+            }
+            LaneRay cameraHit;
+            laneRayInit(cameraHit, cameraO, cameraD, PATHED_TNEAR, PATHED_TFAR, false);
+            unsigned int candidatesLow = 0, candidatesHigh = 0;
+            if (kMasks) {
+                if (got) {
+                    const unsigned long long pixelCandidates = cameraMasks(p)[unitPixel];
+                    candidatesLow = (unsigned int)(pixelCandidates >> 32);
+                    candidatesHigh = (unsigned int)pixelCandidates;
+                }
+            } else if (got) {
+                if (QUADS || MFMA) {
+                    unsigned int unusedLow = 0, unusedHigh = 0;
+                    smallCandidatesItems<false, true, true>(smallTris.data, p.smallQuads, nTris, p.smallKappaT, cameraO, cameraD, cameraD,
+                                                             &candidatesLow, &candidatesHigh, &unusedLow, &unusedHigh, candidateNear(PATHED_TNEAR), 0.f);
+                } else {
+                    smallCandidates(smallTris.data, nTris, cameraO, cameraD, &candidatesLow, &candidatesHigh, candidateNear(PATHED_TNEAR));
+                }
+            }
+            if (COUNT && got) {
+                trisTested += (unsigned int)nTris;
+                closestRays++;
+            }
+            smallResolve(geometry, cameraHit, candidatesLow, candidatesHigh);
+            if (got) { finishRay(geometry, cameraHit); }
+            const bool left = SINGLE && got && cameraHit.bestPrim < 0;
+            const unsigned long long queuedMask = SINGLE ? __ballot(got && !left) : gotMask;
+            SHADE_REGION(8, left);
+            if (got) {
+                const unsigned int slot = (queueHead + queueCount + laneRank(queuedMask)) & (kCameraQueueEntries - 1u);
+                const unsigned int target = singleSample ? (unsigned int)partialIndex(p, newUnit) : newUnit;
+                if (left) {
+                    putUnitAway(p, true, cameraMissColor<TRAITS>(scene, cameraD), target);
+                } else {
+                    cameraQueue[0 * kCameraQueueEntries + slot] = make_float4(cameraD.x, cameraD.y, cameraD.z, cameraHit.best);
+                    cameraQueue[1 * kCameraQueueEntries + slot] = make_float4(cameraHit.bestU, cameraHit.bestV, intAsFloat(cameraHit.bestPrim), intAsFloat((int)target));
+                    cameraQueue[2 * kCameraQueueEntries + slot] = make_float4(intAsFloat((int)cameraRandom.k0), intAsFloat((int)cameraRandom.k1), 0.f, 0.f);
+                }
+            }
+            queueCount += (unsigned int)__popcll(queuedMask);
+            __threadfence_block();
+        }
+
+        const bool tracing = alive && !needEntry;
+        LaneRay ray;
+        laneRayInit(ray, path.o, path.d, PATHED_TNEAR, PATHED_TFAR, false);
+        {
+            const bool traceShadow = tracing && pendingShadow;
+            LaneRay shadowRay;
+            laneRayInit(shadowRay, path.o, shadowDirection, PATHED_TNEAR, shadowTfar, true);
+            unsigned int candidatesLow = 0, candidatesHigh = 0, shadowLow = 0, shadowHigh = 0;
+            SHADE_REGION(2, traceShadow);
+            if (MFMA) {
+                mfmaCandidatesPair(mfmaRows, nTris, p.mfmaFrame, __ballot(traceShadow) != 0ull, path.o, path.d, shadowDirection,
+                                   candidateNear(PATHED_TNEAR), candidateFar(shadowTfar), &candidatesLow, &candidatesHigh, &shadowLow, &shadowHigh);
+                if (!tracing) { candidatesLow = 0u; candidatesHigh = 0u; }
+                if (!traceShadow) { shadowLow = 0u; shadowHigh = 0u; }
+            } else if (QUADS) {
+                if (tracing) {
+                    constexpr bool kPrune = kSmallPrunes<COUNT, TRAITS>;
+                    const int smallQuads = kPassList ? (p.smallQuads & 0xFF) : kPrune ? (p.smallQuads & 0xFFFF) : p.smallQuads;
+                    const int passTris = kPassList ? ((p.smallQuads >> 8) & 0xFF) : nTris;
+                    smallCandidatesItems<true, true, true, kPrune>(smallTris.data, smallQuads, passTris, p.smallKappaT, path.o, path.d, shadowDirection,
+                                                                   &candidatesLow, &candidatesHigh, &shadowLow, &shadowHigh,
+                                                                   candidateNear(PATHED_TNEAR), candidateFar(shadowTfar),
+                                                                   (p.smallQuads >> 16) & 0xFF, (p.smallQuads >> 24) & 0xFF);
+                    if (!traceShadow) { shadowLow = 0u; shadowHigh = 0u; }
+                }
+            } else if (__ballot(traceShadow) != 0ull) {
+                if (tracing) {
+                    smallCandidatesPair(smallTris.data, nTris, path.o, path.d, shadowDirection, &candidatesLow, &candidatesHigh, &shadowLow, &shadowHigh,
+                                        candidateNear(PATHED_TNEAR), candidateFar(shadowTfar));
+                    if (!traceShadow) { shadowLow = 0u; shadowHigh = 0u; }
+                }
+            } else if (tracing) {
+                smallCandidates(smallTris.data, nTris, path.o, path.d, &candidatesLow, &candidatesHigh, candidateNear(PATHED_TNEAR));
+            }
+            if (COUNT && tracing) {
+                trisTested += (unsigned int)nTris * (traceShadow ? 2u : 1u);
+                closestRays++;
+                if (traceShadow) { shadowRays++; }
+            }
+            bool spheresDone = false;
+            RESOLVE_PROBE(9, candidatesLow, candidatesHigh);
+            RESOLVE_PROBE(10, shadowLow, shadowHigh);
+            if (MFMA) {
+                mfmaResolve(geometry, ray, candidatesLow, candidatesHigh);
+                mfmaResolve(geometry, shadowRay, shadowLow, shadowHigh);
+            } else if (QUADS && PATHED_RESOLVE_SHARED) {
+                ResolveScratch scratch;
+                const int waveBase = (int)(threadIdx.x & ~63u), wave = (int)(threadIdx.x >> 6);
+                scratch.best = resolveBest + waveBase; scratch.uv = resolveUv + wave * kResolveCapacity; scratch.items = resolveItems + wave * kResolveCapacity;
+                scratch.occluded = resolveOccluded + waveBase; scratch.count = resolveCount + wave;
+                unsigned int sphereCandidates = 0u, shadowSphereCandidates = 0u;
+                if (TRAITS::spheres && geometry.nSpheres > 0 && tracing) {
+                    smallSphereCandidates(p, geometry.nSpheres, path.o, path.d, shadowDirection, &sphereCandidates, &shadowSphereCandidates);
+                    if (!traceShadow) { shadowSphereCandidates = 0u; }
+                }
+                spheresDone = smallResolveShared<kResolveCapacity, PATHED_RESOLVE_SHARED != 2, TRAITS::spheres>(
+                    passGeometry, ray, shadowRay, candidatesLow, candidatesHigh, shadowLow, shadowHigh, sphereCandidates, shadowSphereCandidates, scratch);
+            } else {
+                smallResolve(passGeometry, ray, candidatesLow, candidatesHigh);
+                smallResolve(passGeometry, shadowRay, shadowLow, shadowHigh);
+            }
+            if (tracing && !spheresDone) { finishRay(geometry, ray); }
+            if (traceShadow) {
+                if (!spheresDone) { finishRay(geometry, shadowRay); }
+                if (shadowRay.occluded) { path.pend = rgb(0.f); }
+            }
+            pendingShadow = false;
+        }
+        if (QUADS) {
+            asm volatile("" ::: "memory");
+            const float4 *stash = stashRows + threadIdx.x;
+            const float4 s0 = stash[0 * kBlock], s1 = stash[1 * kBlock], s2 = stash[2 * kBlock], s4 = stash[(SINGLE ? 2 : 4) * kBlock], s5 = stash[kStashKeyRow * kBlock];
+            path.result = rgb(0.f); path.result.r = s0.x; path.result.g = s0.y; path.result.b = s0.z; path.bsdfPdf = s0.w;
+            path.modulation.r = s1.x; path.modulation.g = s1.y; path.modulation.b = s1.z; path.cosTheta = s1.w;
+            path.throughput.r = s2.x; path.throughput.g = s2.y; path.throughput.b = s2.z; path.st = floatAsInt(s2.w);
+            if (SINGLE) {
+                unit = (unsigned int)floatAsInt(s5.w);
+            } else {
+                partial = stash[3 * kBlock];
+                pixel = (uint32_t)floatAsInt(s4.x); sample = (uint32_t)floatAsInt(s4.y); endSample = (uint32_t)floatAsInt(s4.z); unit = (unsigned int)floatAsInt(s4.w);
+                path.random.dimension = (uint32_t)floatAsInt(s5.w);
+            }
+            path.random.k0 = (uint32_t)floatAsInt(s5.x); path.random.k1 = (uint32_t)floatAsInt(s5.y); path.firstEmitMaterial = floatAsInt(s5.z);
+        }
+        float4 h = make_float4(ray.best, ray.bestU, ray.bestV, intAsFloat(ray.bestPrim));
+
+        bool done = false;
+        bool departs = false;
+        Rgb color = rgb(0.f);
+        if (tracing) {
+            const bool miss = floatAsInt(h.w) < 0;
+            Isect arrived;
+            SHADE_REGION(3, !miss);
+            if (!miss) { arrived = makeIsect<TRAITS>(scene, path.o, path.d, h); }
+            done = pathArrive<TRAITS, true>(p, scene, materials, path, arrived, miss, &color);
+            departs = !done;
+        }
+
+        if (SINGLE) {
+            SHADE_REGION(8, done);
+            putUnitAway(p, done, color, unit);
+            needEntry = needEntry || done;
+            const unsigned long long wanting = __ballot(needEntry);
+            if (wanting != 0ull && queueCount != 0u) {
+                __threadfence_block();
+                const unsigned int rank = laneRank(wanting);
+                if (needEntry && rank < queueCount) {
+                    const unsigned int slot = (queueHead + rank) & (kCameraQueueEntries - 1u);
+                    const float4 e0 = cameraQueue[0 * kCameraQueueEntries + slot];
+                    const float4 e1 = cameraQueue[1 * kCameraQueueEntries + slot];
+                    const float4 e2 = cameraQueue[2 * kCameraQueueEntries + slot];
+                    resetPath(path);
+                    path.o = cameraOrigin(scene.camera);
+                    path.d = v3(e0.x, e0.y, e0.z);
+                    path.random.k0 = (uint32_t)floatAsInt(e2.x); path.random.k1 = (uint32_t)floatAsInt(e2.y); path.random.dimension = 2u;
+                    h = make_float4(e0.w, e1.x, e1.y, e1.z);
+                    unit = (unsigned int)floatAsInt(e1.w);
+                    needEntry = false;
+                    departs = true;
+                }
+                const unsigned int wanted = (unsigned int)__popcll(wanting);
+                const unsigned int taken = wanted < queueCount ? wanted : queueCount;
+                queueHead = (queueHead + taken) & (kCameraQueueEntries - 1u);
+                queueCount -= taken;
+            }
+            if (queueCount == 0u && !unitsLeft && needEntry) { alive = false; needEntry = false; }
+        } else while (true) {
+            SHADE_REGION(8, done);
+            {
+                const bool unitDone = putSampleAway(p, singleSample, done, color, partial, unit, sample, endSample);
+                needEntry = needEntry || unitDone;
+                startNext = startNext || (done && !unitDone);
+            }
+            done = false;
+            const unsigned long long wanting = __ballot(needEntry);
+            if (wanting == 0ull) { break; }
+            if (queueCount == 0u) {
+                if (!unitsLeft && needEntry) { alive = false; needEntry = false; }
+                break;
+            }
+            __threadfence_block();
+            const unsigned int rank = laneRank(wanting);
+            if (needEntry && rank < queueCount) {
+                const unsigned int slot = (queueHead + rank) & (kCameraQueueEntries - 1u);
+                const float4 e0 = cameraQueue[0 * kCameraQueueEntries + slot];
+                const float4 e1 = cameraQueue[1 * kCameraQueueEntries + slot];
+                const float4 e2 = cameraQueue[2 * kCameraQueueEntries + slot];
+                resetPath(path);
+                path.o = cameraOrigin(scene.camera);
+                path.d = v3(e0.x, e0.y, e0.z);
+                path.random.k0 = (uint32_t)floatAsInt(e2.x); path.random.k1 = (uint32_t)floatAsInt(e2.y); path.random.dimension = 2u;
+                h = make_float4(e0.w, e1.x, e1.y, e1.z);
+                unit = (unsigned int)floatAsInt(e1.w);
+                if (singleSample) { sample = 0u; endSample = 1u; }
+                else { unitSamples(p, unit, &pixel, &sample, &endSample); }
+                needEntry = false;
+                if (floatAsInt(h.w) < 0) {
+                    color = cameraMissColor<TRAITS>(scene, path.d);
+                    done = true;
+                } else {
+                    departs = true;
+                }
+            }
+            const unsigned int wanted = (unsigned int)__popcll(wanting);
+            const unsigned int taken = wanted < queueCount ? wanted : queueCount;
+            queueHead = (queueHead + taken) & (kCameraQueueEntries - 1u);
+            queueCount -= taken;
+        }
+        if (__ballot(alive) == 0ull) { break; }
+
+        SHADE_REGION(6, departs);
+        bool ended = false;
+        if (departs) {
+            uint32_t keyRow[kKeyRowWords] = {};
+            if (SINGLE) {
+                const int vertex = (path.st & kStBounceMask) + 1;
+                const int table = keySlots.find(path.random.k1);
+                if (table >= 0 && vertex <= kKeyVertices) {
+                    const uint4 *row = keyTables + (table * kKeyTableWords + (vertex - 1) * kKeyRowWords) / 4;
+                    const uint4 low = row[0], high = row[1];
+                    keyRow[0] = low.x; keyRow[1] = low.y; keyRow[2] = low.z; keyRow[3] = low.w;
+                    keyRow[4] = high.x; keyRow[5] = high.y; keyRow[6] = high.z; keyRow[7] = high.w;
+                } else {
+                    fillKeyRow(path.random.k1, vertex, keyRow);
+                }
+            }
+            Isect isect = makeIsect<TRAITS>(scene, path.o, path.d, h);
+            ShadowRequest shadow;
+            ended = pathDepart<TRAITS, true, SINGLE>(p, scene, materials, path, isect, &shadow, &color, keyRow);
+            if (shadow.push) {
+                pendingShadow = true;
+                shadowDirection = shadow.direction;
+                shadowTfar = shadow.tfar;
+            }
+        }
+        if (__ballot(ended) != 0ull) {
+            SHADE_REGION(8, ended);
+            if (SINGLE) {
+                putUnitAway(p, ended, color, unit);
+                needEntry = needEntry || ended;
+            } else {
+                const bool unitDone = putSampleAway(p, singleSample, ended, color, partial, unit, sample, endSample);
+                needEntry = needEntry || unitDone;
+                startNext = startNext || (ended && !unitDone);
+            }
+        }
+    }
+
+    if (COUNT) {
+        atomicAdd(&p.stats[kStatTris], (unsigned long long)trisTested);
+        atomicAdd(&p.stats[kStatClosest], (unsigned long long)closestRays);
+        atomicAdd(&p.stats[kStatShadow], (unsigned long long)shadowRays);
+    }
diff --git a/pathed_amd/csrc/pathed_hip.hip b/pathed_amd/csrc/pathed_hip.hip
--- a/pathed_amd/csrc/pathed_hip.hip
+++ b/pathed_amd/csrc/pathed_hip.hip
@@ -2156,6 +2156,7 @@
                 } else if (kSmallPrunes<decltype(COUNT)::value, TRAITS>) {
                     params.smallQuads = scene->smallLayout.nQuads | scene->smallLayout.shadowQuadPairs << 16 | scene->smallLayout.shadowLonePairs << 24;
                 }
+                if (!decltype(COUNT)::value && std::is_same<TRAITS, TraitsLambertianTriangles>::value && params.chunk == 1) { return k_path_small_single; }
                 return k_path_small<true, decltype(COUNT)::value, TRAITS, false, true>;
             };
             const std::false_type plain{};
diff --git a/pathed_amd/csrc/shading.h b/pathed_amd/csrc/shading.h
--- a/pathed_amd/csrc/shading.h
+++ b/pathed_amd/csrc/shading.h
@@ -46,7 +46,7 @@
     uint32_t k0, k1;
     uint32_t dimension;
 
-    __device__ inline float next()
+    __host__ __device__ inline float next()
     {
         const uint32_t bits = mix32(k0 + mix32(k1 + dimension * 0x9e3779b9u));
         dimension++;
@@ -60,7 +60,54 @@
     *k1 = mix32(sample ^ mix32((uint32_t)(seed >> 32) ^ 0x9e3779b9u));
 }
 
-__device__ inline uint32_t vertexBase(int vertex) { return 2u + 8u * (uint32_t)(vertex - 1); }
+__host__ __device__ inline uint32_t vertexBase(int vertex) { return 2u + 8u * (uint32_t)(vertex - 1); }
+
+static const int kKeyVertices = 12;
+static const int kKeyRowWords = 8;
+static const int kKeyTableWords = kKeyVertices * kKeyRowWords;
+
+__host__ __device__ inline uint32_t innerKey(uint32_t k1, uint32_t dimension) { return mix32(k1 + dimension * 0x9e3779b9u); }
+
+__host__ __device__ inline void fillKeyRow(uint32_t k1, int vertex, uint32_t *row)
+{
+    for (int j = 0; j < kKeyRowWords; j++) { row[j] = innerKey(k1, vertexBase(vertex) + (uint32_t)j); }
+}
+
+__host__ __device__ inline float drawFromRow(uint32_t k0, const uint32_t *row, uint32_t column)
+{
+    const uint32_t bits = mix32(k0 + row[column]);
+    return (float)(bits >> 8) * 5.9604638e-08f;
+}
+
+struct RowRng {
+    uint32_t k0;
+    const uint32_t *row;
+    uint32_t dimension;
+
+    __host__ __device__ inline float next() { return drawFromRow(k0, row, dimension++); }
+};
+
+struct KeySlots {
+    uint32_t tag[2];
+    uint32_t filled;
+    uint32_t older;
+
+    __host__ __device__ inline void clear() { tag[0] = 0u; tag[1] = 0u; filled = 0u; older = 0u; }
+    __host__ __device__ inline int find(uint32_t k1) const
+    {
+        if ((filled & 1u) != 0u && tag[0] == k1) { return 0; }
+        if ((filled & 2u) != 0u && tag[1] == k1) { return 1; }
+        return -1;
+    }
+    __host__ __device__ inline int claim(uint32_t k1)
+    {
+        const int slot = (filled & 1u) == 0u ? 0 : (filled & 2u) == 0u ? 1 : (int)older;
+        if (slot == 0) { tag[0] = k1; } else { tag[1] = k1; }
+        filled |= 1u << slot;
+        older = (uint32_t)(slot ^ 1);
+        return slot;
+    }
+};
 
 
 struct Frame {
```
